# CMU-SAFARI/Scrooge

Hardware: AMD Instinct MI355X
Metric: aligned pairs/s (+ GCUPS) at W=64, 10kb reads; 1/2/4/8 MI355X (higher is better)
Workload: dtype u64

## Files before the change

### scrooge_amd/csrc/genasm_lane_kernel.hip

```cpp

#include <hip/hip_runtime.h>
#include <stdint.h>
#include <type_traits>

#include "lane_common.h"

namespace scrg {

constexpr int LANE_TB_COLS = 31;
constexpr uint32_t LANE_RING_BYTES = 68;
constexpr uint32_t LANE_SCRATCH_BYTES = 36;
constexpr uint32_t LANE_EQ_BYTES = 32;
constexpr uint32_t LANE_NOMATCH_BYTES = 8;
constexpr uint32_t LANE_WAVE_LDS_BYTES = 64u * (LANE_RING_BYTES + LANE_SCRATCH_BYTES + LANE_EQ_BYTES + LANE_NOMATCH_BYTES);
constexpr uint32_t LANE_EQ_SLOT_STRIDE = 512;
constexpr uint32_t LANE_EQ_REGION_BYTES = 4u * LANE_EQ_SLOT_STRIDE;
constexpr uint32_t LANE_EQ_FIELD_MASK = 3u * LANE_EQ_SLOT_STRIDE;
constexpr uint32_t LANE_REST_BYTES = LANE_WAVE_LDS_BYTES - LANE_EQ_REGION_BYTES;
constexpr int LANE_EQ_AHEAD = 8;

__device__ __forceinline__ uint32_t lane_read_offset(uint32_t fwd_offset, uint32_t read_idx, uint32_t read_len, uint32_t revm)
{
    return bitop3<TT_BFI>(sub_sat_u32(read_len - read_idx, 64u), fwd_offset, revm);
}
__device__ __forceinline__ void lane_pattern_rev(const Planes pw, uint32_t left, uint32_t revm, bool any_rev, uint64_t& rlo, uint64_t& rhi)
{
    rlo = brev64(pw.lo);
    rhi = brev64(pw.hi);
    if (any_rev) {
        const uint32_t sh = sub_sat_u32(64u, left);
        const uint64_t flo = ~(pw.lo << sh), fhi = ~(pw.hi << sh);
        rlo = ((uint64_t)bitop3<TT_BFI>((uint32_t)(flo >> 32), (uint32_t)(rlo >> 32), revm) << 32) | bitop3<TT_BFI>((uint32_t)flo, (uint32_t)rlo, revm);
        rhi = ((uint64_t)bitop3<TT_BFI>((uint32_t)(fhi >> 32), (uint32_t)(rhi >> 32), revm) << 32) | bitop3<TT_BFI>((uint32_t)fhi, (uint32_t)rhi, revm);
    }
}

constexpr uint32_t LANE_TEXT_REV = 1u << 7;
__device__ __forceinline__ uint32_t lane_text_offset(uint32_t ref_idx, uint32_t text_len, uint32_t tr_in)
{
    return bitop3<TT_BFI>(text_rev_at(text_len, ref_idx, 0u).at, ref_idx, neg_mask(tr_in << 24));
}
__device__ __forceinline__ void lane_text_rev(Planes& tw, uint32_t text_len, uint32_t ref_idx, uint32_t tr_in)
{
    const uint32_t tm = neg_mask(tr_in << 24);
    const uint32_t sh = text_rev_at(text_len, ref_idx, 0u).sh;
    const uint64_t flo = ~brev64(tw.lo << sh), fhi = ~brev64(tw.hi << sh);
    tw.lo = ((uint64_t)bitop3<TT_BFI>((uint32_t)(flo >> 32), (uint32_t)(tw.lo >> 32), tm) << 32) | bitop3<TT_BFI>((uint32_t)flo, (uint32_t)tw.lo, tm);
    tw.hi = ((uint64_t)bitop3<TT_BFI>((uint32_t)(fhi >> 32), (uint32_t)(tw.hi >> 32), tm) << 32) | bitop3<TT_BFI>((uint32_t)fhi, (uint32_t)tw.hi, tm);
}

template <bool NOMATCH>
__device__ __forceinline__ void lane_write_eq(const uint64_t rlo, const uint64_t rhi, const uint32_t iv0, const uint32_t iv1,
                                              const uint32_t eq_b, const uint32_t nomatch_b)
{
    const uint32_t rl0 = (uint32_t)rlo, rl1 = (uint32_t)(rlo >> 32), rh0 = (uint32_t)rhi, rh1 = (uint32_t)(rhi >> 32);
    lds_write64(eq_b, make_uint2(~(rl0 | rh0) | iv0, ~(rl1 | rh1) | iv1));
    lds_write64(eq_b + LANE_EQ_SLOT_STRIDE, make_uint2((rl0 & ~rh0) | iv0, (rl1 & ~rh1) | iv1));
    lds_write64(eq_b + 2u * LANE_EQ_SLOT_STRIDE, make_uint2((~rl0 & rh0) | iv0, (~rl1 & rh1) | iv1));
    lds_write64(eq_b + 3u * LANE_EQ_SLOT_STRIDE, make_uint2((rl0 & rh0) | iv0, (rl1 & rh1) | iv1));
    if (NOMATCH) lds_write64(nomatch_b, make_uint2(iv0, iv1));
}
struct LaneEqAddr {
    uint32_t xe0, xo0, xe1, xo1, eq_b;
    __device__ __forceinline__ LaneEqAddr(const Planes tw, const uint32_t eq_b_) : eq_b(eq_b_)
    {
        const uint32_t tl0 = (uint32_t)tw.lo, tl1 = (uint32_t)(tw.lo >> 32), th0 = (uint32_t)tw.hi, th1 = (uint32_t)(tw.hi >> 32);
        xe0 = bitop3<TT_BFI>(tl0, th0 << 1, 0x55555555u), xo0 = bitop3<TT_BFI>(th0, tl0 >> 1, 0xaaaaaaaau);
        xe1 = bitop3<TT_BFI>(tl1, th1 << 1, 0x55555555u), xo1 = bitop3<TT_BFI>(th1, tl1 >> 1, 0xaaaaaaaau);
    }
    __device__ __forceinline__ uint32_t at(const int i) const
    {
        const int b = i & 31;
        const uint32_t x = (b & 1) ? (i < 32 ? xo0 : xo1) : (i < 32 ? xe0 : xe1);
        const int f = (b & 1) ? b - 1 : b;
        const uint32_t u = f >= 9 ? x >> (f - 9) : x << (9 - f);
        return bitop3<TT_ANDOR>(u, LANE_EQ_FIELD_MASK, eq_b);
    }
};

template <bool SHORT_N>
__device__ __forceinline__ void lane_window_table(const Planes tw, const uint64_t rlo, const uint64_t rhi, const uint32_t n, const uint32_t m,
                                                  const uint32_t stop, uint64_t (&tab)[LANE_TB_COLS],
                                                  const uint32_t eq_b, const uint32_t nomatch_b, const bool write_eq = true)
{
    const uint64_t valid = ~0ull << (64u - m);
    const uint32_t iv0 = ~(uint32_t)valid, iv1 = ~(uint32_t)(valid >> 32);
    if (write_eq) lane_write_eq<SHORT_N>(rlo, rhi, iv0, iv1, eq_b, nomatch_b);
    const LaneEqAddr ea(tw, eq_b);
    auto eq_addr = [&](int i) -> uint32_t {
        const uint32_t a = ea.at(i);
        if (!SHORT_N) return a;
        return bitop3<TT_BFI>(a, nomatch_b, neg_mask((uint32_t)i - n));
    };
    uint2 eqw[LANE_EQ_AHEAD];
#pragma unroll
    for (int k = 0; k < LANE_EQ_AHEAD; k++) eqw[k] = lds_read64(eq_addr(63 - k));
    uint32_t pv0 = (uint32_t)valid, pv1 = (uint32_t)(valid >> 32), mv0 = 0u, mv1 = 0u;
#pragma unroll
    for (int i = 63; i >= 0; i--) {
        const uint2 eq_now = eqw[(63 - i) % LANE_EQ_AHEAD];
        if (i - LANE_EQ_AHEAD >= 0) eqw[(63 - i) % LANE_EQ_AHEAD] = lds_read64(eq_addr(i - LANE_EQ_AHEAD));
        {
            const uint32_t eq0 = eq_now.x, eq1 = eq_now.y;
            const uint32_t xv0 = eq0 | mv0, xv1 = eq1 | mv1;
            const uint32_t t0 = eq0 & pv0, t1 = eq1 & pv1;
            const uint64_t sum = add64(((uint64_t)t1 << 32) | t0, ((uint64_t)pv1 << 32) | pv0);
            const uint32_t xh0 = bitop3<TT_XH>((uint32_t)sum, pv0, eq0), xh1 = bitop3<TT_XH>((uint32_t)(sum >> 32), pv1, eq1);
            const uint32_t ph0 = bitop3<TT_PH>(mv0, xh0, pv0), ph1 = bitop3<TT_PH>(mv1, xh1, pv1);
            const uint32_t mh0 = pv0 & xh0, mh1 = pv1 & xh1;
            const uint64_t phs = shl1(((uint64_t)ph1 << 32) | ph0);
            const uint64_t mhs = shl1(((uint64_t)mh1 << 32) | mh0);
            pv0 = bitop3<TT_PVN>((uint32_t)mhs, xv0, (uint32_t)phs);
            pv1 = bitop3<TT_PVN>((uint32_t)(mhs >> 32), xv1, (uint32_t)(phs >> 32));
            mv0 = (uint32_t)phs & xv0;
            mv1 = (uint32_t)(phs >> 32) & xv1;
            if (i < LANE_TB_COLS)
                tab[i] = ((uint64_t)bitop3<TT_NOR3>(pv1, ph1, stop) << 32) | bitop3<TT_V0>(pv1, ph1, xh1);
        }
    }
}

constexpr int BAND_UP = 10, BAND_DOWN = 21, BAND_SAFE = 19;
static_assert(BAND_UP + BAND_DOWN + 1 == 32 && BAND_SAFE / 2 + 1 <= BAND_UP && BAND_SAFE + 1 <= BAND_DOWN, "the band holds every cell a safe walk asks about");
constexpr int TT_D0 = bitop3_table([](int sum, int pv, int xv) { return (sum ^ pv) | xv; });
constexpr int TT_OR3 = bitop3_table([](int a, int b, int c) { return a | b | c; });
constexpr int TT_NIV_BAND = bitop3_table([](int v1, int v0, int stop) { return ~(v1 & v0) | stop; });
__device__ __forceinline__ uint64_t lane_band_stop0(const uint32_t TBL)
{
    uint64_t s0 = 0x8000000000000000ull >> (TBL + (uint32_t)BAND_UP - 1u);
    asm volatile("" : "+s"(s0));
    return s0;
}
__device__ __forceinline__ uint32_t lane_band_stop(const uint64_t stop0, const int i)
{
    return (uint32_t)((stop0 << i) >> 32);
}
constexpr bool LANE_BAND_TABLE = true;
constexpr uint32_t BAND_STRETCH = 32, BAND_REDO_MAX = 6;
__device__ __forceinline__ uint32_t add_masked(uint32_t acc, const uint32_t x, const uint32_t mask)
{
    uint32_t t;
    asm volatile("v_and_b32 %0, %2, %3\n\tv_add_u32 %1, %1, %0" : "=&v"(t), "+v"(acc) : "s"(mask), "v"(x));
    return acc;
}
__device__ __forceinline__ uint32_t lane_window_table_band(const Planes tw, const uint64_t rlo, const uint64_t rhi, const uint32_t TBL,
                                                           uint64_t (&tab)[LANE_TB_COLS], const uint32_t eq_b)
{
    lane_write_eq<false>(rlo, rhi, 0u, 0u, eq_b, 0u);
    const LaneEqAddr ea(tw, eq_b);
    const uint64_t stop0 = lane_band_stop0(TBL);
    auto band_eq = [&](const uint2 w, const int i) -> uint32_t {
        const int s = 62 - i - BAND_DOWN;
        if (s >= 32) return w.y >> (s - 32);
        if (s > 0) return __builtin_amdgcn_alignbit(w.y, w.x, (uint32_t)s);
        if (s == 0) return w.x;
        return __builtin_amdgcn_alignbit(w.x, 0xffffffffu, (uint32_t)(32 + s));
    };
    uint2 eqw[LANE_EQ_AHEAD];
#pragma unroll
    for (int k = 0; k < LANE_EQ_AHEAD; k++) eqw[k] = lds_read64(ea.at(63 - k));
    uint32_t pv = ~0u << (BAND_DOWN + 1), mv = 0u;
    uint32_t fd = 0u;
#pragma unroll
    for (int i = 63; i >= 0; i--) {
        const uint32_t eq = band_eq(eqw[(63 - i) % LANE_EQ_AHEAD], i);
        if (i - LANE_EQ_AHEAD >= 0) eqw[(63 - i) % LANE_EQ_AHEAD] = lds_read64(ea.at(i - LANE_EQ_AHEAD));
        const uint32_t xv = eq | mv;
        const uint32_t d0 = bitop3<TT_D0>((eq & pv) + pv, pv, xv);
        const uint32_t ph = bitop3<TT_PH>(mv, d0, pv);
        const uint32_t mh = pv & d0;
        fd = add_masked(fd, d0, 1u << (32 - BAND_UP));
        const uint32_t xvs = xv >> 1;
        pv = bitop3<TT_PVN>(mh, xvs, ph);
        mv = ph & xvs;
        if (i < LANE_TB_COLS) {
            uint32_t pv2;
            asm("v_add_u32 %0, %1, %1" : "=v"(pv2) : "v"(pv));
            uint32_t v1 = bitop3<TT_OR3>(pv2, ph, lane_band_stop(stop0, i)), v0 = bitop3<TT_V0>(pv2, ph, d0);
            asm volatile("" : "+v"(v1), "+v"(v0));
            tab[i] = ((uint64_t)v1 << 32) | v0;
        }
    }
    return 64u - (fd >> (32 - BAND_UP));
}

template <int OUT>
__global__ __launch_bounds__(256, 4) void genasm_lane_kernel(AlignArgs a)
{
    constexpr bool EDITS = OUT == LANE_OUT_EDITS, NONE = OUT == LANE_OUT_NONE;
    constexpr bool BAND = LANE_BAND_TABLE;
    constexpr uint32_t REST_BYTES = NONE ? 64u * LANE_NOMATCH_BYTES : LANE_REST_BYTES;
    constexpr uint32_t STAGE_BYTES = NONE ? 0u : 64u * (LANE_RING_BYTES + LANE_SCRATCH_BYTES);
    extern __shared__ __attribute__((aligned(16))) uint32_t lds[];
    char* const lds_b = reinterpret_cast<char*>(lds);

    const uint32_t lane = threadIdx.x & 63u;
    const uint32_t wave = threadIdx.x >> 6, wpg = blockDim.x >> 6;
    const uint32_t wave_b = wpg * LANE_EQ_REGION_BYTES + wave * REST_BYTES;
    const uint32_t ring_b = wave_b + lane * LANE_RING_BYTES;
    const uint32_t scr_b = wave_b + 64u * LANE_RING_BYTES + lane * LANE_SCRATCH_BYTES;
    uint8_t* const lds8 = reinterpret_cast<uint8_t*>(lds);
    const uint32_t lds0 = (uint32_t)(uintptr_t)(__attribute__((address_space(3))) char*)lds_b;
    const uint32_t eq_b = lds0 + wave * LANE_EQ_REGION_BYTES + lane * 8u;
    const uint32_t nomatch_b = lds0 + wave_b + STAGE_BYTES + lane * LANE_NOMATCH_BYTES;
    const uint32_t W = (uint32_t)a.W;
    const uint32_t TBL = (uint32_t)a.tb_limit;

    bool has_pair = false;
    uint32_t pair = 0;
    const uint64_t* text_w = a.seq;
    const uint64_t* read_w = a.seq;
    uint32_t tr_in = 0;
    uint64_t cigar_off = 0;
    uint32_t text_len = 0, read_len = 0, cigar_cap = 0;
    uint32_t ref_idx = 0, read_idx = 0, edits = 0;
    uint32_t lim = 0xffffffffu;
    uint32_t revm = 0;
    int32_t nr = -1;
    uint32_t flushed = 0;
    uint32_t pos = 0;
    uint32_t mbase = 0;
    WindowWords twords = {0, 0, 0, 0}, pwords = {0, 0, 0, 0};
    bool queue_empty = false;
    const bool timing = SCRG_TIMING(a);
    uint64_t cy_fetch = 0, cy_setup = 0, cy_dc = 0, cy_tb = 0, cy_p1 = 0;
    uint32_t st_rounds = 0, st_gen = 0;
    uint32_t band_ctl = 0;
    uint32_t st_band = 0, st_redone = 0, st_skipped = 0;
    const uint64_t rt0 = timing ? __builtin_amdgcn_s_memrealtime() : 0;

    auto write_piece = [&]() {
        if constexpr (!NONE) scrg::write_piece<EDITS>(a, lds, ring_b, cigar_off, cigar_cap, flushed, !SCRG_ABL(a, 16));
    };
    auto flush_pieces = [&]() {
        if constexpr (!NONE) {
            const bool need = has_pair && (EDITS ? pos - flushed >= 32u : nr - (int32_t)flushed >= 15);
            if (__any(need)) {
                if (need) write_piece();
            }
        }
    };
    auto ring_guard = [&](uint32_t fill, uint32_t limit) {
        if (__any(has_pair && fill >= limit)) {
            if (has_pair && fill >= (EDITS ? 32u : 16u)) write_piece();
        }
    };

    uint32_t rot = hw_wave_slot();
    for (;;) {
        if (!SCRG_SW(a, 1)) rotate_priority(rot++);
        const uint64_t tm0 = timing ? __builtin_readcyclecounter() : 0;
        for (;;) {
            const bool over = has_pair && edits > lim;
            const bool fin = over || (has_pair && read_idx >= read_len);
            if (__any(fin)) {
                if (over) abandon_pair<OUT>(a, pair, edits);
                else if constexpr (NONE) { if (fin) retire_pair_distance(a, pair, edits, ref_idx); }
                else if (fin) retire_pair<EDITS>(a, lds, ring_b, pair, cigar_off, cigar_cap, flushed, EDITS ? pos : (uint32_t)(nr + 1), nr, edits, !SCRG_ABL(a, 16));
                has_pair = has_pair && !fin;
            }
            const bool want = !has_pair && !queue_empty;
            if (!__any(want)) break;
            const uint32_t idx = claim_pairs(a, lane, want);
            const bool got = want && idx < a.n_pairs;
            if (__any(want && idx >= a.n_pairs)) queue_empty = true;
            if (got) {
                const scrg_pair_desc pd = a.pairs[idx];
                pair = idx;
                const TextStretch ts = text_stretch(pd.text_off, pd.text_len, a.text_rev != 0u, a.text_stride);
                text_w = a.seq + (ts.off >> 5);
                const uint64_t r_off = a.stranded ? pd.read_off & ~SCRG_READ_REVCOMP : pd.read_off;
                revm = (a.stranded && (pd.read_off & SCRG_READ_REVCOMP)) ? 0xffffffffu : 0u;
                read_w = a.seq + (r_off >> 5);
                tr_in = ((uint32_t)ts.off & 31u) | (((uint32_t)r_off & 31u) << 8) | (ts.rev ? LANE_TEXT_REV : 0u);
                text_len = ts.len;
                read_len = (uint32_t)pd.read_len;
                lim = pair_edit_limit(a, read_len);
                if constexpr (NONE) {
                    ref_idx = read_idx = edits = 0;
                } else {
                    cigar_off = pd.cigar_off;
                    cigar_cap = pd.cigar_cap > 0xffffffffull ? 0xffffffffu : (uint32_t)pd.cigar_cap;
                    ref_idx = read_idx = edits = flushed = pos = mbase = 0;
                    nr = -1;
                }
                has_pair = true;
                twords = load_window_words_at(text_w, tr_in & 31u, ts.rev ? text_rev_at(text_len, 0u, 0u).at : 0u, a.text_stride);
                pwords = load_window_words_at(read_w, tr_in >> 8, lane_read_offset(0u, 0u, read_len, revm), a.read_stride);
            }
        }
        if (!__any(has_pair)) break;
        const bool wave_rev = a.stranded && __any(has_pair && revm != 0u);
        const bool wave_trev = a.text_rev && __any(has_pair && (tr_in & LANE_TEXT_REV) != 0u);

        const uint64_t tm1 = timing ? __builtin_readcyclecounter() : 0;
        const uint32_t n = has_pair ? min(W, sub_sat_u32(text_len, ref_idx)) : 0u;
        const uint32_t m = has_pair ? min(W, read_len - read_idx) : 1u;
        Planes tw = window_planes(twords);
        const Planes pw = window_planes(pwords);
        if (wave_trev) lane_text_rev(tw, text_len, ref_idx, tr_in);
        asm volatile("" :: "v"(tw.lo), "v"(tw.hi), "v"(pw.lo), "v"(pw.hi) : "memory");
        flush_pieces();
        const uint64_t tm2 = timing ? __builtin_readcyclecounter() : 0;

        uint64_t tab[LANE_TB_COLS];
        const uint32_t jlim = has_pair ? min(m, TBL) : 0u;
        const uint32_t stop = 0x80000000u >> jlim;
        const bool short_n = __any(has_pair && n != 64u);
        uint64_t rlo, rhi;
        lane_pattern_rev(pw, read_len - read_idx, revm, wave_rev, rlo, rhi);
        uint32_t j = 0, ti, nDm = 0, Xm = 0, nIm = 0;
        auto walk = [&](auto full_tag, auto band_tag) {
            constexpr bool FULL = decltype(full_tag)::value;
            constexpr bool BANDED = decltype(band_tag)::value;
            const uint64_t stop0 = BANDED ? lane_band_stop0(TBL) : 0ull;
#pragma unroll
            for (int i = 0; i < LANE_TB_COLS; i++) {
                if (!FULL && (uint32_t)i >= TBL) continue;
                const uint32_t x = (BANDED ? bitop3<TT_NIV_BAND>((uint32_t)(tab[i] >> 32), (uint32_t)tab[i], lane_band_stop(stop0, i))
                                           : bitop3<TT_NIV>((uint32_t)(tab[i] >> 32), (uint32_t)tab[i], stop)) << j;
                const uint32_t ni = ffbh_u32(x);
                if constexpr (!NONE) lds_store_u8(lds0 + scr_b + (uint32_t)i, ni);
                nIm = __builtin_amdgcn_alignbit(nIm, x, 31);
                j += ni;
                const uint64_t both = tab[i] << j;
                const uint32_t nt1 = (uint32_t)(both >> 32), t0 = (uint32_t)both;
                nDm = __builtin_amdgcn_alignbit(nDm, nt1, 31);
                Xm = __builtin_amdgcn_alignbit(Xm, t0, 31);
                if (BANDED) j += neg_mask(nt1);
                else j -= neg_mask(nt1);
            }
        };
        bool walked = false, eq_written = false;
        uint64_t tm3 = 0;
        if constexpr (BAND) {
            if (W == 64u && !short_n && !__any(has_pair && m != 64u) && !SCRG_SEL(a.debug, SCRG_SWITCH_NO_BAND) && !SCRG_ABL(a, 2) && !SCRG_ABL(a, 8)) {
                if ((band_ctl >> 16) != 0u) {
                    band_ctl -= 1u << 16;
                    st_skipped++;
                } else {
                    const uint32_t d_band = lane_window_table_band(tw, rlo, rhi, TBL, tab, eq_b);
                    walked = !__any(has_pair && d_band > (uint32_t)BAND_SAFE);
                    eq_written = true;
                    st_band++;
                    st_redone += walked ? 0u : 1u;
                    band_ctl += walked ? 1u : 0x101u;
                    if (((band_ctl >> 8) & 15u) > BAND_REDO_MAX && !SCRG_SEL(a.debug, SCRG_SWITCH_BAND_ALWAYS)) {
                        const uint32_t fails = (band_ctl >> 12) & 15u;
                        band_ctl = (32u << (16u + fails)) | (min(fails + 1u, 6u) << 12);
                    } else if ((band_ctl & 255u) == BAND_STRETCH) {
                        band_ctl = 0u;
                    }
                    if (walked) {
                        tm3 = timing ? __builtin_readcyclecounter() : 0;
                        j = (uint32_t)BAND_UP - 1u;
                        if (TBL == (uint32_t)LANE_TB_COLS) walk(std::true_type{}, std::true_type{});
                        else walk(std::false_type{}, std::true_type{});
                        j = has_pair ? j + TBL - ((uint32_t)BAND_UP - 1u) : 0u;
                        nDm = has_pair ? ~nDm : 0u;
                        nIm = has_pair ? nIm : ~0u;
                    }
                }
            }
        }
        if (!walked) {
            if (SCRG_ABL(a, 2)) {
#pragma unroll
                for (int i = 0; i < LANE_TB_COLS; i++) tab[i] = ((uint64_t)~stop << 32) | (((uint32_t)tw.lo * (uint32_t)(i + 1)) | stop);
            } else if (short_n) {
                lane_window_table<true>(tw, rlo, rhi, n, m, stop, tab, eq_b, nomatch_b);
                st_gen++;
            } else {
                lane_window_table<false>(tw, rlo, rhi, n, m, stop, tab, eq_b, nomatch_b, !eq_written);
            }
            tm3 = timing ? __builtin_readcyclecounter() : 0;
            if (SCRG_ABL(a, 8)) { j = jlim; nDm = ~0u; }
            else if (TBL == (uint32_t)LANE_TB_COLS) walk(std::true_type{}, std::false_type{});
            else walk(std::false_type{}, std::false_type{});
        }
        {
            if (timing) cy_p1 += __builtin_readcyclecounter() - tm3;
            const uint32_t TBc = min(TBL, (uint32_t)LANE_TB_COLS);
            const uint32_t nsh = 32u - TBc;
            const uint32_t notD = nDm << nsh, Xraw = Xm << nsh;
            const uint32_t Draw = ~notD;
            const uint32_t Im = ~nIm << nsh;
            const uint32_t ti_stopped = (31u - ffbl_u32((notD >> 1) | Im)) & 31u;
            ti = bitop3<TT_BFI>(TBc, ti_stopped, neg_mask(j - jlim));
            const uint32_t A = ~(0xffffffffu >> ti);
            const uint32_t D = Draw & A, X = Xraw & A;
            const uint32_t B = ((D ^ (D >> 1)) | (X ^ (X >> 1)) | Im | 0x80000000u) & A;
            const uint32_t nD = (uint32_t)__builtin_popcount(D), nX = (uint32_t)__builtin_popcount(X);
            edits += j - ti + 2u * nD + nX;
            ref_idx += ti;
            read_idx += j;
            twords = load_window_words_at(text_w, tr_in & 31u, wave_trev ? lane_text_offset(ref_idx, text_len, tr_in) : ref_idx, a.text_stride);
            const uint32_t left_x = read_idx ^ read_len;
            const uint32_t fwd_at = read_idx & neg_mask(left_x | (0u - left_x));
            pwords = load_window_words_at(read_w, tr_in >> 8, wave_rev ? lane_read_offset(fwd_at, read_idx, read_len, revm) : fwd_at, a.read_stride);

            if constexpr (NONE) {
                (void)B;
            } else if constexpr (EDITS) {
                uint32_t E = SCRG_ABL(a, 4) ? 0u : (D | X | Im);
                nr += (int32_t)(__builtin_popcount(B) + __builtin_popcount(Im));
                uint32_t c = ffbh_u32(E);
                uint32_t ni = lds8[scr_b + c];
                auto put = [&](uint32_t at, uint32_t b) { lds8[ring_b + (at & 63u)] = (uint8_t)b; };
                auto event = [&]() {
                    const uint32_t sh = 31u - c;
                    const uint32_t bit = 0x80000000u >> (c & 31u);
                    uint32_t iB = __builtin_amdgcn_ubfe(Im, sh, 1), dx = __builtin_amdgcn_ubfe(D | X, sh, 1);
                    const uint32_t xB = __builtin_amdgcn_ubfe(X, sh, 1);
                    const uint32_t t = mbase + c;
                    E = bitop3<TT_ANDN>(E, bit, bit);
                    const uint32_t nx = ffbh_u32(E);
                    const uint32_t step = 0xC0u - 0x80u * xB;
                    const bool side = ni * iB > 3u;
                    if (__any(side)) {
                        if (side) {
                            auto emit = [&](uint32_t b) {
                                put(pos, b);
                                pos++;
                                if (pos - flushed >= 32u) write_piece();
                            };
                            emit(0x80u | t);
                            for (uint32_t q = 1; q < ni; q++) emit(0x80u);
                            mbase = 0u - c;
                            if (dx) {
                                emit(step);
                                mbase = ~c;
                            }
                            iB = dx = 0;
                        }
                    }
                    put(pos, 0x80u | t);
                    put(pos + 1u, 0x80u);
                    put(pos + 2u, 0x80u);
                    pos += iB ? ni : 0u;
                    put(pos, step | (iB ? 0u : t));
                    pos += dx;
                    mbase = dx ? ~c : (iB ? 0u - c : mbase);
                    ni = lds8[scr_b + nx];
                    c = nx;
                };
                uint32_t trips = 0;
                while (__any(E != 0u)) {
                    if (trips >= 2u) ring_guard(pos - flushed, 50u);
                    event();
                    event();
                    trips++;
                }
                put(pos, mbase + ti);
                pos += has_pair ? 1u : 0u;
                mbase = 0;
            } else {
            uint32_t E = SCRG_ABL(a, 4) ? 0u : (B | Im);
            uint32_t c0 = ffbh_u32(E);
            E = bitop3<TT_ANDN>(E, 0x80000000u >> (c0 & 31u), 0u);
            uint32_t c1 = ffbh_u32(E);
            uint32_t q = 2u * (uint32_t)nr + 2u;
            auto event = [&](uint32_t& c, const uint32_t ni, const uint32_t nx) {
                const uint32_t sh = 31u - c;
                const uint32_t aI = ring_b + (q & 62u);
                q = add_twice(q, __builtin_amdgcn_ubfe(Im, sh, 1));
                const uint32_t w = add3(mad24(__builtin_amdgcn_ubfe(X, sh, 1), 27u << 8, mad24(__builtin_amdgcn_ubfe(D, sh, 1), 7u << 8, sh)),
                                        min(nx, ti), ((uint32_t)'=' << 8) - 31u);
                const uint32_t aS = ring_b + (q & 62u);
                q = add_twice(q, __builtin_amdgcn_ubfe(B, sh, 1));
                E = bitop3<TT_ANDN>(E, 0x80000000u >> (nx & 31u), 0u);
                c = ffbh_u32(E);
                *reinterpret_cast<uint16_t*>(lds_b + aI) = (uint16_t)(((uint32_t)'I' << 8) | ni);
                *reinterpret_cast<uint16_t*>(lds_b + aS) = (uint16_t)w;
            };
            auto trip = [&]() {
                const uint32_t n0 = lds8[scr_b + c0], n1 = lds8[scr_b + c1];
                event(c0, n0, c1);
                event(c1, n1, c0);
            };
            for (uint32_t trips = 0; trips < 4u && __any(c0 < 32u); trips++) trip();
            while (__any(c0 < 32u)) {
                ring_guard((q >> 1) - flushed, 27u);
                trip();
            }
            nr = ((int32_t)q >> 1) - 1;
            }
        }
        st_rounds++;
        if (timing) {
            const uint64_t tm4 = __builtin_readcyclecounter();
            cy_fetch += tm1 - tm0;
            cy_setup += tm2 - tm1;
            cy_dc += tm3 - tm2;
            cy_tb += tm4 - tm3;
        }
    }
    if (timing && lane == 0) {
        atomicAdd((unsigned long long*)&a.stats[0], (unsigned long long)st_rounds | ((unsigned long long)st_skipped << 32));
        atomicAdd((unsigned long long*)&a.stats[1], (unsigned long long)st_gen | ((unsigned long long)st_band << 21) | ((unsigned long long)st_redone << 42));
        atomicAdd((unsigned long long*)&a.stats[2], (unsigned long long)cy_p1);
        atomicAdd((unsigned long long*)&a.stats[3], (unsigned long long)cy_fetch);
        atomicAdd((unsigned long long*)&a.stats[4], (unsigned long long)cy_setup);
        atomicAdd((unsigned long long*)&a.stats[5], (unsigned long long)cy_dc);
        atomicAdd((unsigned long long*)&a.stats[6], (unsigned long long)cy_tb);
        const uint64_t rt1 = __builtin_amdgcn_s_memrealtime();
        atomicAdd((unsigned long long*)&a.stats[7], (unsigned long long)(rt1 - rt0));
        atomicMax((unsigned long long*)&a.stats[8], (unsigned long long)rt0);
        atomicMax((unsigned long long*)&a.stats[9], (unsigned long long)((1ull << 62) - rt0));
        atomicMax((unsigned long long*)&a.stats[10], (unsigned long long)rt1);
        atomicMax((unsigned long long*)&a.stats[11], (unsigned long long)((1ull << 62) - rt1));
    }
}

constexpr uint32_t SPLIT_FIELDS = 6;
constexpr uint32_t SPLIT_BUF_BYTES = SPLIT_FIELDS * 256u + 64u * LANE_SCRATCH_BYTES;
constexpr uint32_t SPLIT_PAIR_LDS_BYTES = 64u * (LANE_RING_BYTES + LANE_EQ_BYTES + LANE_NOMATCH_BYTES) + 2u * SPLIT_BUF_BYTES;
constexpr uint32_t SPLIT_WG_LDS_BYTES = 4u * SPLIT_PAIR_LDS_BYTES + 64u;
constexpr uint32_t SPLIT_VALID = 1u << 8, SPLIT_FIRST = 1u << 9, SPLIT_LAST = 1u << 10;
constexpr uint32_t SPLIT_OVER = 1u << 11;

__global__ __launch_bounds__(512, 2) void genasm_lane_split_kernel(AlignArgs a)
{
    extern __shared__ __attribute__((aligned(16))) uint32_t lds[];
    char* const lds_b = reinterpret_cast<char*>(lds);
    uint8_t* const lds8 = reinterpret_cast<uint8_t*>(lds);
    const uint32_t lane = threadIdx.x & 63u;
    const uint32_t wave = threadIdx.x >> 6, duo = wave & 3u;
    const bool consumer = wave >= 4u;
    const uint32_t duo_b = 4u * LANE_EQ_REGION_BYTES + duo * (SPLIT_PAIR_LDS_BYTES - LANE_EQ_REGION_BYTES);
    const uint32_t ring_b = duo_b + lane * LANE_RING_BYTES;
    const uint32_t lds0 = (uint32_t)(uintptr_t)(__attribute__((address_space(3))) char*)lds_b;
    const uint32_t eq_b = lds0 + duo * LANE_EQ_REGION_BYTES + lane * 8u;
    const uint32_t nomatch_b = lds0 + duo_b + 64u * LANE_RING_BYTES + lane * LANE_NOMATCH_BYTES;
    const uint32_t bufs_b = duo_b + 64u * (LANE_RING_BYTES + LANE_NOMATCH_BYTES);
    const uint32_t flags_w = (4u * SPLIT_PAIR_LDS_BYTES) >> 2;
    const uint32_t W = (uint32_t)a.W;
    const uint32_t TBL = (uint32_t)a.tb_limit;
    const uint32_t TBc = min(TBL, (uint32_t)LANE_TB_COLS);
    const uint32_t nsh = 32u - TBc;
    auto rec_w = [&](uint32_t buf, uint32_t field) -> uint32_t { return ((bufs_b + buf * SPLIT_BUF_BYTES) >> 2) + field * 64u + lane; };
    auto len_b = [&](uint32_t buf) -> uint32_t { return bufs_b + buf * SPLIT_BUF_BYTES + SPLIT_FIELDS * 256u + lane * LANE_SCRATCH_BYTES; };
    auto all_done = [&](uint32_t r) -> bool {
        const uint32_t f = flags_w + (r & 1u) * 4u;
        return (lds[f] & lds[f + 1] & lds[f + 2] & lds[f + 3]) != 0u;
    };

    if (!consumer) {
        bool has_pair = false, active = true;
        uint32_t pair = 0;
        uint64_t text_off = 0, read_off = 0;
        uint32_t text_len = 0, read_len = 0;
        uint32_t ref_idx = 0, read_idx = 0, edits = 0;
        uint32_t lim = 0xffffffffu;
        uint32_t revm = 0;
        bool trev = false;
        WindowWords twords = {0, 0, 0, 0}, pwords = {0, 0, 0, 0};
        bool queue_empty = false;
        uint32_t st_rounds = 0;
        const uint32_t slot = hw_wave_slot();
        for (uint32_t r = 0;; r++) {
            const uint32_t buf = r & 1u;
            uint32_t first = 0;
            if (active) {
                if (!SCRG_SW(a, 1)) rotate_priority(r + slot);
                has_pair = has_pair && read_idx < read_len && edits <= lim;
                for (;;) {
                    const bool want = !has_pair && !queue_empty;
                    if (!__any(want)) break;
                    const uint32_t idx = claim_pairs(a, lane, want);
                    const bool got = want && idx < a.n_pairs;
                    if (__any(want && idx >= a.n_pairs)) queue_empty = true;
                    if (got) {
                        const LanePair p = unpack_pair(a, idx);
                        pair = idx;
                        text_off = p.text_off;
                        read_off = p.read_off;
                        revm = p.rev ? 0xffffffffu : 0u;
                        trev = p.trev;
                        text_len = p.text_len;
                        read_len = p.read_len;
                        lim = pair_edit_limit(a, p.read_len);
                        ref_idx = read_idx = edits = 0;
                        has_pair = true;
                        first = SPLIT_FIRST;
                        twords = load_window_words(a.seq, text_off, trev ? text_rev_at(text_len, 0u, 0u).at : 0u, a.text_stride);
                        pwords = load_window_words(a.seq, read_off, lane_read_offset(0u, 0u, read_len, revm), a.read_stride);
                    }
                }
                if (!__any(has_pair)) active = false;
            }
            if (active) {
                const bool live = has_pair && read_idx < read_len;
                const uint32_t n = (live && ref_idx < text_len) ? min(W, text_len - ref_idx) : 0u;
                const uint32_t m = live ? min(W, read_len - read_idx) : 1u;
                Planes tw = {0, 0}, pw = {0, 0};
                if (live) {
                    tw = window_planes(twords);
                    pw = window_planes(pwords);
                }
                const bool wave_trev = a.text_rev && __any(live && trev);
                if (wave_trev) lane_text_rev(tw, text_len, ref_idx, trev ? LANE_TEXT_REV : 0u);
                uint64_t tab[LANE_TB_COLS];
                const uint32_t jlim = live ? min(m, TBL) : 0u;
                const uint32_t stop = 0x80000000u >> jlim;
                const bool short_n = __any(live && n != 64u);
                const bool wave_rev = a.stranded && __any(live && revm != 0u);
                uint64_t rlo, rhi;
                lane_pattern_rev(pw, read_len - read_idx, revm, wave_rev, rlo, rhi);
                if (short_n) lane_window_table<true>(tw, rlo, rhi, n, m, stop, tab, eq_b, nomatch_b);
                else lane_window_table<false>(tw, rlo, rhi, n, m, stop, tab, eq_b, nomatch_b);
                uint32_t j = 0, nDm = 0, Xm = 0, nIm = 0;
                const uint32_t lb = len_b(buf);
                auto walk = [&](auto full_tag) {
                    constexpr bool FULL = decltype(full_tag)::value;
#pragma unroll
                    for (int i = 0; i < LANE_TB_COLS; i++) {
                        if (!FULL && (uint32_t)i >= TBL) continue;
                        const uint32_t x = bitop3<TT_NIV>((uint32_t)(tab[i] >> 32), (uint32_t)tab[i], stop) << j;
                        const uint32_t ni = ffbh_u32(x);
                        lds_store_u8(lds0 + lb + (uint32_t)i, ni);
                        nIm = __builtin_amdgcn_alignbit(nIm, x, 31);
                        j += ni;
                        const uint64_t both = tab[i] << j;
                        const uint32_t nt1 = (uint32_t)(both >> 32), t0 = (uint32_t)both;
                        nDm = __builtin_amdgcn_alignbit(nDm, nt1, 31);
                        Xm = __builtin_amdgcn_alignbit(Xm, t0, 31);
                        j -= neg_mask(nt1);
                    }
                };
                if (TBL == (uint32_t)LANE_TB_COLS) walk(std::true_type{});
                else walk(std::false_type{});
                const uint32_t notD = nDm << nsh, Xraw = Xm << nsh;
                const uint32_t Im = ~nIm << nsh;
                const uint32_t ti_stopped = (31u - ffbl_u32((notD >> 1) | Im)) & 31u;
                const uint32_t ti = bitop3<TT_BFI>(TBc, ti_stopped, neg_mask(j - jlim));
                const uint32_t A = ~(0xffffffffu >> ti);
                const uint32_t D = ~notD & A, X = Xraw & A;
                edits += j - ti + 2u * (uint32_t)__builtin_popcount(D) + (uint32_t)__builtin_popcount(X);
                ref_idx += ti;
                read_idx += j;
                twords = load_window_words(a.seq, text_off, wave_trev ? lane_text_offset(ref_idx, text_len, trev ? LANE_TEXT_REV : 0u) : ref_idx, a.text_stride);
                const uint32_t left_x = read_idx ^ read_len;
                pwords = load_window_words(a.seq, read_off, lane_read_offset(read_idx & neg_mask(left_x | (0u - left_x)), read_idx, read_len, revm), a.read_stride);
                const uint32_t over = (has_pair && edits > lim) ? SPLIT_OVER : 0u;
                const uint32_t last = (has_pair && (read_idx >= read_len || over)) ? SPLIT_LAST : 0u;
                lds[rec_w(buf, 0)] = D;
                lds[rec_w(buf, 1)] = X;
                lds[rec_w(buf, 2)] = Im;
                lds[rec_w(buf, 3)] = ti | (has_pair ? SPLIT_VALID : 0u) | first | last | over;
                lds[rec_w(buf, 4)] = pair;
                lds[rec_w(buf, 5)] = edits;
                st_rounds++;
            } else {
                lds[rec_w(buf, 3)] = 0u;
            }
            if (lane == 0) lds[flags_w + buf * 4u + duo] = active ? 0u : 1u;
            __syncthreads();
            if (all_done(r)) break;
        }
        if (SCRG_TIMING(a) && lane == 0) atomicAdd((unsigned long long*)&a.stats[0], (unsigned long long)st_rounds);
        return;
    }

    bool open = false;
    uint32_t pair = 0;
    uint64_t cigar_off = 0;
    uint32_t cigar_cap = 0;
    int32_t nr = -1;
    uint32_t flushed = 0;
    auto flush_pieces = [&]() {
        const bool need = open && nr - (int32_t)flushed >= 16;
        if (__any(need)) {
            if (need) write_piece<false>(a, lds, ring_b, cigar_off, cigar_cap, flushed);
        }
    };
    auto consume = [&](uint32_t buf) {
        const uint32_t meta = lds[rec_w(buf, 3)];
        if (!__any((meta & SPLIT_VALID) != 0u)) return;
        const bool valid = (meta & SPLIT_VALID) != 0u;
        const uint32_t ti = meta & 31u;
        const uint32_t D = valid ? lds[rec_w(buf, 0)] : 0u, X = valid ? lds[rec_w(buf, 1)] : 0u, Im = valid ? lds[rec_w(buf, 2)] : 0u;
        if (valid && (meta & SPLIT_FIRST)) {
            pair = lds[rec_w(buf, 4)];
            const LanePair p = unpack_pair(a, pair);
            cigar_off = p.cigar_off;
            cigar_cap = p.cigar_cap;
            nr = -1;
            flushed = 0;
            open = true;
        }
        const uint32_t A = ~(0xffffffffu >> ti);
        const uint32_t B = ((D ^ (D >> 1)) | (X ^ (X >> 1)) | Im | 0x80000000u) & A;
        const uint32_t scr_b = len_b(buf);
        uint32_t E = valid ? (B | Im) : 0u;
        uint32_t c = ffbh_u32(E);
        uint32_t ni = lds8[scr_b + c];
        uint32_t q = 2u * (uint32_t)nr + 2u;
        auto event = [&]() {
            const uint32_t sh = 31u - c;
            const uint32_t bit = 0x80000000u >> (c & 31u);
            *reinterpret_cast<uint16_t*>(lds_b + ring_b + (q & 62u)) = (uint16_t)(((uint32_t)'I' << 8) | ni);
            q = add_twice(q, __builtin_amdgcn_ubfe(Im, sh, 1));
            E = bitop3<TT_ANDN>(E, bit, bit);
            const uint32_t nx = ffbh_u32(E);
            ni = lds8[scr_b + nx];
            const uint32_t w = add3(mad24(__builtin_amdgcn_ubfe(X, sh, 1), 27u << 8, mad24(__builtin_amdgcn_ubfe(D, sh, 1), 7u << 8, sh)),
                                    min(nx, ti), ((uint32_t)'=' << 8) - 31u);
            *reinterpret_cast<uint16_t*>(lds_b + ring_b + (q & 62u)) = (uint16_t)w;
            q = add_twice(q, __builtin_amdgcn_ubfe(B, sh, 1));
            c = nx;
        };
        uint32_t trips = 0;
        while (__any(E != 0u)) {
            event();
            event();
            if (++trips == 3u) {
                trips = 0;
                nr = ((int32_t)q >> 1) - 1;
                flush_pieces();
            }
        }
        nr = ((int32_t)q >> 1) - 1;
        flush_pieces();
        const bool fin = valid && (meta & SPLIT_LAST) != 0u;
        if (__any(fin)) {
            if (fin && (meta & SPLIT_OVER)) {
                abandon_pair<LANE_OUT_RUNS>(a, pair, lds[rec_w(buf, 5)]);
                open = false;
            } else if (fin) {
                const uint32_t n_runs = (uint32_t)(nr + 1);
                while (n_runs - flushed >= 16u) write_piece<false>(a, lds, ring_b, cigar_off, cigar_cap, flushed);
                const uint32_t rem = n_runs - flushed;
                const uint32_t rd = (ring_b >> 2) + ((flushed & 16u) >> 1);
                uint32_t* const dst = reinterpret_cast<uint32_t*>(a.runs + cigar_off + flushed);
                for (uint32_t k = 0; 2u * k < rem; k++)
                    if (flushed + 2u * k < cigar_cap) dst[k] = lds[rd + k];
                a.ed[pair] = (int64_t)lds[rec_w(buf, 5)];
                a.n_runs[pair] = n_runs;
                a.status[pair] = n_runs > cigar_cap ? LANE_STATUS_OVERFLOW : LANE_STATUS_DONE;
                open = false;
            }
        }
    };
    for (uint32_t r = 0;; r++) {
        if (r != 0u) consume((r - 1u) & 1u);
        __syncthreads();
        if (all_done(r)) {
            consume(r & 1u);
            break;
        }
    }
}

hipError_t launch_align_lane_split(const AlignArgs& a, int grid, hipStream_t s)
{
    const dim3 g((grid + 3) / 4), b(512);
    hipLaunchKernelGGL(genasm_lane_split_kernel, g, b, SPLIT_WG_LDS_BYTES, s, a);
    return hipGetLastError();
}

hipError_t launch_align_lane(const AlignArgs& a, int grid, size_t lds_bytes, hipStream_t s, LaneOutput out)
{
    const unsigned wpg = SCRG_SW(a, 64) ? 1u : (SCRG_SW(a, 128) ? 2u : 4u);
    const dim3 g((grid + wpg - 1) / wpg), b(64 * wpg);
    with_lane_output(out, [&](auto o) { hipLaunchKernelGGL(genasm_lane_kernel<decltype(o)::value>, g, b, wpg * lds_bytes, s, a); });
    return hipGetLastError();
}

}
```

### scrooge_amd/csrc/genasm_lane_mw_kernel.hip

```cpp

#include <hip/hip_runtime.h>
#include <stdint.h>

#include "lane_multiword.h"
#include "row_ops.h"

namespace scrg {

namespace {

constexpr uint32_t MW_RING_BYTES = 68;

}

template <int NW, int RW, int OUT>
__global__ __launch_bounds__(64) void genasm_lane_mw_kernel(AlignArgs a)
{
    extern __shared__ __attribute__((aligned(16))) uint32_t lds[];
    char* const lds_b = reinterpret_cast<char*>(lds);
    uint8_t* const lds8 = reinterpret_cast<uint8_t*>(lds);

    constexpr bool EDITS = OUT == LANE_OUT_EDITS, NONE = OUT == LANE_OUT_NONE;
    const uint32_t lane = threadIdx.x;
    const uint32_t W = (uint32_t)a.W;
    const uint32_t TBL = (uint32_t)a.tb_limit;
    const uint32_t ring_b = lane * MW_RING_BYTES;
    const uint32_t len_b = 64u * MW_RING_BYTES + lane * lane_mw_len_bytes(a.tb_limit);
    uint64_t* const tab = reinterpret_cast<uint64_t*>(a.spill) + (uint64_t)blockIdx.x * (uint64_t)TBL * 2u * RW * 64u + lane;

    bool rev = false;
    bool trev = false;
    LaneWork lp;

    auto write_piece = [&]() {
        if constexpr (!NONE) scrg::write_piece<EDITS>(a, lds, ring_b, lp.cigar_off, lp.cigar_cap, lp.flushed);
    };
    auto flush_pieces = [&]() {
        for (;;) {
            const bool need = lp.has_pair && lp.nr + 1 - (int32_t)lp.flushed >= 16;
            if (!__any(need)) break;
            if (need) write_piece();
        }
    };
    auto push_run = [&](uint32_t op, uint32_t count) {
        lp.nr++;
        *reinterpret_cast<uint16_t*>(lds_b + ring_b + (((uint32_t)lp.nr & 31u) << 1)) = (uint16_t)(count | (op << 8));
    };
    auto emit = [&](uint32_t b) {
        lds8[ring_b + (lp.pos & 63u)] = (uint8_t)b;
        lp.pos++;
        if (lp.pos - lp.flushed >= 32u) write_piece();
    };

    for (;;) {
        if (!next_pairs<OUT, !EDITS>(a, lds, ring_b, lane, lp, rev, trev)) break;

        const uint32_t n = (lp.has_pair && lp.ref_idx < lp.text_len) ? min(W, lp.text_len - lp.ref_idx) : 0u;
        const uint32_t m = lp.has_pair ? min(W, lp.read_len - lp.read_idx) : 1u;
        uint64_t tlo[NW], thi[NW], rlo[NW], rhi[NW], valid[NW];
        const bool wave_trev = a.text_rev && __any(lp.has_pair && trev);
#pragma unroll
        for (int w = 0; w < NW; w++) {
            Planes t = {0, 0}, p = {0, 0};
            if (lp.has_pair && !trev && 64u * (uint32_t)w < n) t = load_window_strided(a.seq, lp.text_off, lp.ref_idx + 64u * (uint32_t)w, a.text_stride);
            if (wave_trev) {
                if (lp.has_pair && trev && 64u * (uint32_t)w < n) t = text_revcomp_word(a.seq, lp.text_off, lp.text_len, lp.ref_idx, (uint32_t)w, a.text_stride);
            }
            if (lp.has_pair && 64u * (uint32_t)w < m) p = load_window_strided(a.seq, lp.read_off, lp.read_idx + 64u * (uint32_t)w, a.read_stride);
            tlo[w] = t.lo;
            thi[w] = t.hi;
            rlo[w] = brev64(p.lo);
            rhi[w] = brev64(p.hi);
            if (a.stranded && __any(lp.has_pair && rev)) {
                const Planes rv = revcomp_pattern_word(a.seq, lp.read_off, lp.read_len, lp.has_pair ? lp.read_idx : lp.read_len, (uint32_t)w, a.read_stride);
                if (lp.has_pair && rev) { rlo[w] = rv.lo; rhi[w] = rv.hi; }
            }
            const uint32_t lo = 64u * (uint32_t)w;
            valid[w] = m >= lo + 64u ? ~0ull : (m <= lo ? 0ull : ~0ull << (64u - (m - lo)));
        }
        const uint32_t jlim = lp.has_pair ? min(m, TBL) : 0u;
        const Row<RW> stop = row_bit<RW>(jlim);

        {
            uint64_t pv[NW], mv[NW];
#pragma unroll
            for (int w = 0; w < NW; w++) { pv[w] = valid[w]; mv[w] = 0; }
#pragma unroll
            for (int wi = NW - 1; wi >= 0; wi--) {
                for (int b = 63; b >= 0; b--) {
                    const uint32_t i = 64u * (uint32_t)wi + (uint32_t)b;
                    if (i >= W) continue;
                    const uint64_t sl = 0ull - ((tlo[wi] >> b) & 1ull), sh = 0ull - ((thi[wi] >> b) & 1ull);
                    const bool in_text = i < n;
                    uint64_t xv[NW], xh[NW], ph[NW], mh[NW];
                    uint64_t carry = 0;
#pragma unroll
                    for (int w = NW - 1; w >= 0; w--) {
                        const uint64_t eq = (in_text ? ~((rlo[w] ^ sl) | (rhi[w] ^ sh)) : 0ull) | ~valid[w];
                        xv[w] = eq | mv[w];
                        const uint64_t t = eq & pv[w];
                        const uint64_t s1 = t + pv[w];
                        const uint64_t s2 = s1 + carry;
                        carry = (uint64_t)(s1 < t) | (uint64_t)(s2 < s1);
                        xh[w] = (s2 ^ pv[w]) | eq;
                        ph[w] = mv[w] | ~(xh[w] | pv[w]);
                        mh[w] = pv[w] & xh[w];
                    }
#pragma unroll
                    for (int w = 0; w < NW; w++) {
                        const uint64_t ph1 = (ph[w] << 1) | (w + 1 < NW ? ph[w + 1] >> 63 : 0ull);
                        const uint64_t mh1 = (mh[w] << 1) | (w + 1 < NW ? mh[w + 1] >> 63 : 0ull);
                        pv[w] = mh1 | ~(xv[w] | ph1);
                        mv[w] = ph1 & xv[w];
                    }
                    if (i < TBL) {
#pragma unroll
                        for (int r = 0; r < RW; r++) {
                            const uint64_t pvr = r < NW ? pv[r < NW ? r : 0] : 0ull, phr = r < NW ? ph[r < NW ? r : 0] : 0ull, xhr = r < NW ? xh[r < NW ? r : 0] : ~0ull;
                            tab[((uint64_t)(i * 2u) * RW + r) * 64u] = ~((pvr | phr) | stop.w[r]);
                            tab[((uint64_t)(i * 2u + 1u) * RW + r) * 64u] = (pvr | ~(phr | xhr)) | stop.w[r];
                        }
                    }
                }
            }
        }

        {
            uint32_t j = 0;
            Row<RW> nDm = row_zero<RW>(), Xm = row_zero<RW>(), nIm = row_zero<RW>();
            constexpr int CH = RW == 1 ? 16 : (RW == 2 ? 8 : 4);
            for (uint32_t i0 = 0; i0 < TBL; i0 += CH) {
                Row<RW> nv1[CH], v0[CH];
#pragma unroll
                for (int q = 0; q < CH; q++) {
                    const uint32_t i = min(i0 + (uint32_t)q, TBL - 1u);
#pragma unroll
                    for (int r = 0; r < RW; r++) {
                        nv1[q].w[r] = tab[((uint64_t)(i * 2u) * RW + r) * 64u];
                        v0[q].w[r] = tab[((uint64_t)(i * 2u + 1u) * RW + r) * 64u];
                    }
                }
#pragma unroll
                for (int q = 0; q < CH; q++) {
                    const uint32_t i = i0 + (uint32_t)q;
                    if (i >= TBL) continue;
                    Row<RW> x;
#pragma unroll
                    for (int r = 0; r < RW; r++) x.w[r] = nv1[q].w[r] | ~v0[q].w[r] | stop.w[r];
                    x = row_shl<RW>(x, j);
                    const uint32_t ni = row_clz<RW>(x);
                    if constexpr (!NONE) lds8[len_b + i] = (uint8_t)ni;
                    nIm = row_shl1_in<RW>(nIm, x.w[0] >> 63);
                    j += ni;
                    const Row<RW> nt1 = row_shl<RW>(nv1[q], j), t0 = row_shl<RW>(v0[q], j);
                    nDm = row_shl1_in<RW>(nDm, nt1.w[0] >> 63);
                    Xm = row_shl1_in<RW>(Xm, t0.w[0] >> 63);
                    j += (uint32_t)(nt1.w[0] >> 63);
                }
            }
            const uint32_t nsh = 64u * RW - TBL;
            Row<RW> Draw = row_shl<RW>(nDm, nsh), Im;
            const Row<RW> Xraw = row_shl<RW>(Xm, nsh);
#pragma unroll
            for (int r = 0; r < RW; r++) { Draw.w[r] = ~Draw.w[r]; Im.w[r] = ~nIm.w[r]; }
            Im = row_shl<RW>(Im, nsh);
            const Row<RW> lim = row_bit<RW>(TBL);
            Row<RW> dead;
#pragma unroll
            for (int r = 0; r < RW; r++) dead.w[r] = (Draw.w[r] & Xraw.w[r]) | lim.w[r];
            const uint32_t ti = row_clz<RW>(dead);
            const Row<RW> A = row_top<RW>(ti);
            Row<RW> D, X, B, E;
#pragma unroll
            for (int r = 0; r < RW; r++) { D.w[r] = Draw.w[r] & A.w[r]; X.w[r] = Xraw.w[r] & A.w[r]; }
            const Row<RW> D1 = row_shr1<RW>(D), X1 = row_shr1<RW>(X);
#pragma unroll
            for (int r = 0; r < RW; r++) {
                B.w[r] = ((D.w[r] ^ D1.w[r]) | (X.w[r] ^ X1.w[r]) | Im.w[r] | (r == 0 ? TOP : 0ull)) & A.w[r];
                E.w[r] = B.w[r] | Im.w[r];
            }
            lp.edits += j - ti + 2u * row_pop<RW>(D) + row_pop<RW>(X);
            lp.ref_idx += ti;
            lp.read_idx += j;

            if constexpr (NONE) {
            } else if constexpr (EDITS) {
                Row<RW> Ev;
#pragma unroll
                for (int r = 0; r < RW; r++) Ev.w[r] = D.w[r] | X.w[r] | Im.w[r];
                lp.nr += (int32_t)(row_pop<RW>(B) + row_pop<RW>(Im));
                while (__any(row_any<RW>(Ev))) {
                    if (row_any<RW>(Ev)) {
                        const uint32_t c = row_clz<RW>(Ev);
                        const Row<RW> bit = row_bit<RW>(c);
#pragma unroll
                        for (int r = 0; r < RW; r++) Ev.w[r] &= ~bit.w[r];
                        uint32_t t = lp.mbase + c;
                        if (row_test<RW>(Im, c)) {
                            const uint32_t ni = lds8[len_b + c];
                            for (; t >= 63u; t -= 63u) emit(0x3Fu);
                            emit(0x80u | t);
                            for (uint32_t q = 1; q < ni; q++) emit(0x80u);
                            t = 0;
                            lp.mbase = 0u - c;
                        }
                        const bool isD = row_test<RW>(D, c), isX = row_test<RW>(X, c);
                        if (isD || isX) {
                            for (; t >= 63u; t -= 63u) emit(0x3Fu);
                            emit((isX ? 0x40u : 0xC0u) | t);
                            lp.mbase = ~c;
                        }
                    }
                }
                if (__any(lp.has_pair)) {
                    if (lp.has_pair) {
                        uint32_t t = lp.mbase + ti;
                        for (; t >= 63u; t -= 63u) emit(0x3Fu);
                        emit(t);
                    }
                }
                lp.mbase = 0;
            } else
            while (__any(row_any<RW>(E))) {
                if (row_any<RW>(E)) {
                    const uint32_t c = row_clz<RW>(E);
                    if (row_test<RW>(Im, c)) push_run((uint32_t)'I', lds8[len_b + c]);
                    const Row<RW> bit = row_bit<RW>(c);
#pragma unroll
                    for (int r = 0; r < RW; r++) E.w[r] &= ~bit.w[r];
                    const uint32_t nx = min(row_clz<RW>(E), ti);
                    if (row_test<RW>(B, c))
                        push_run(row_test<RW>(D, c) ? (uint32_t)'D' : (row_test<RW>(X, c) ? (uint32_t)'X' : (uint32_t)'='), nx - c);
                }
                flush_pieces();
            }
        }
    }
}

template <int NW, int RW> static hipError_t launch_mw(const AlignArgs& a, int grid, size_t lds_bytes, hipStream_t s, LaneOutput out)
{
    with_lane_output(out, [&](auto o) { hipLaunchKernelGGL((genasm_lane_mw_kernel<NW, RW, decltype(o)::value>), dim3(grid), dim3(64), lds_bytes, s, a); });
    return hipGetLastError();
}

hipError_t launch_align_lane_mw(const AlignArgs& a, int grid, size_t lds_bytes, hipStream_t s, LaneOutput out)
{
    const int nw = a.W <= 64 ? 1 : (a.W <= 128 ? 2 : 4), rw = a.tb_limit / 64 + 1;
    if (nw == 1 && rw == 1) return launch_mw<1, 1>(a, grid, lds_bytes, s, out);
    if (nw == 1 && rw == 2) return launch_mw<1, 2>(a, grid, lds_bytes, s, out);
    if (nw == 2 && rw == 3) return launch_mw<2, 3>(a, grid, lds_bytes, s, out);
    if (nw == 2 && rw == 1) return launch_mw<2, 1>(a, grid, lds_bytes, s, out);
    if (nw == 2 && rw == 2) return launch_mw<2, 2>(a, grid, lds_bytes, s, out);
    if (nw == 4 && rw == 1) return launch_mw<4, 1>(a, grid, lds_bytes, s, out);
    if (nw == 4 && rw == 2) return launch_mw<4, 2>(a, grid, lds_bytes, s, out);
    if (nw == 4 && rw == 3) return launch_mw<4, 3>(a, grid, lds_bytes, s, out);
    if (nw == 4 && rw == 4) return launch_mw<4, 4>(a, grid, lds_bytes, s, out);
    return hipErrorInvalidValue;
}

}
```

### scrooge_amd/csrc/genasm_lane_parts_kernel.hip

```cpp

#include <hip/hip_runtime.h>
#include <stdint.h>
#include <type_traits>

#include "lane_multiword.h"

namespace scrg {

namespace {

constexpr int PT_COLS = 16;
constexpr uint32_t PT_RING_BYTES = 68;
constexpr uint32_t PT_SCRATCH_BYTES = 20;
constexpr int PT_EQ_AHEAD = 2;

__device__ __forceinline__ uint64_t pt_from_row(uint64_t w0, uint64_t w1, uint32_t s)
{
    const bool far = s >= 64u;
    const uint64_t hi = far ? w1 : w0, lo = far ? 0ull : w1;
    const uint32_t b = s & 63u;
    return shl64(hi, b) | shr64(lo >> 1, 63u - b);
}

template <int NW, bool STORE, bool SHORT>
__device__ __forceinline__ void pt_sweep16(LaneVec<NW>& st, const uint32_t xe, const uint32_t xo, const int32_t nrel, const uint2 (&stop)[2],
                                           uint64_t (&tab)[PT_COLS][2][2], const uint32_t eq_b, const uint32_t nomatch_b)
{
    constexpr int SLOT_SHIFT = NW == 2 ? 4 : 5;
    auto eq_addr = [&](int c) -> uint32_t {
        const uint32_t x = (c & 1) ? xo : xe;
        const int f = (c & 1) ? c - 1 : c;
        const uint32_t u = f >= SLOT_SHIFT ? x >> (f - SLOT_SHIFT) : x << (SLOT_SHIFT - f);
        const uint32_t a = bitop3<TT_ANDOR>(u, 3u << SLOT_SHIFT, eq_b);
        return (!SHORT || c < nrel) ? a : nomatch_b;
    };
    uint2 eqw[PT_EQ_AHEAD][NW];
#pragma unroll
    for (int k = 0; k < PT_EQ_AHEAD; k++) {
        const uint32_t ad = eq_addr(PT_COLS - 1 - k);
#pragma unroll
        for (int q = 0; q < NW; q++) eqw[k][q] = lds_read64(ad + 8u * q);
    }
#pragma unroll
    for (int c = PT_COLS - 1; c >= 0; c--) {
        uint2 eq[NW];
#pragma unroll
        for (int q = 0; q < NW; q++) eq[q] = eqw[(PT_COLS - 1 - c) % PT_EQ_AHEAD][q];
        if (c - PT_EQ_AHEAD >= 0) {
            const uint32_t ad = eq_addr(c - PT_EQ_AHEAD);
#pragma unroll
            for (int q = 0; q < NW; q++) eqw[(PT_COLS - 1 - c) % PT_EQ_AHEAD][q] = lds_read64(ad + 8u * q);
        }
        const LaneColumn<NW> col = sweep_column<NW>(st, eq);
        if (STORE) {
#pragma unroll
            for (int r = 0; r < 2; r++) {
                table_words<NW>(st, col, r, stop[r], tab[c][0][r], tab[c][1][r]);
            }
        }
    }
}

}

template <int NW, int OUT>
__global__ __launch_bounds__(256, 2) void genasm_lane_parts_kernel(AlignArgs a)
{
    extern __shared__ __attribute__((aligned(16))) uint32_t lds[];
    char* const lds_b = reinterpret_cast<char*>(lds);
    uint8_t* const lds8 = reinterpret_cast<uint8_t*>(lds);
    constexpr uint32_t SLOT = NW == 2 ? 16u : 32u;
    constexpr uint32_t EQ_BYTES = 4u * SLOT, NOMATCH_BYTES = SLOT, TEXT_BYTES = 16u * NW;
    constexpr bool EDITS = OUT == LANE_OUT_EDITS, NONE = OUT == LANE_OUT_NONE;
    constexpr uint32_t STAGE_BYTES = NONE ? 0u : PT_RING_BYTES + PT_SCRATCH_BYTES;
    constexpr uint32_t WAVE_LDS = 64u * (STAGE_BYTES + EQ_BYTES + NOMATCH_BYTES + TEXT_BYTES);
    constexpr uint32_t CP_DWORDS = 4u * NW;

    const uint32_t lane = threadIdx.x & 63u;
    const uint32_t wave_b = (threadIdx.x >> 6) * WAVE_LDS;
    const uint32_t ring_b = wave_b + lane * PT_RING_BYTES;
    const uint32_t scr_b = wave_b + 64u * PT_RING_BYTES + lane * PT_SCRATCH_BYTES;
    const uint32_t eq_base = (uint32_t)(uintptr_t)(__attribute__((address_space(3))) char*)lds_b + wave_b + 64u * STAGE_BYTES;
    const uint32_t eq_b = eq_base + lane * EQ_BYTES;
    const uint32_t nomatch_b = eq_base + 64u * EQ_BYTES + lane * NOMATCH_BYTES;
    const uint32_t text_b = eq_base + 64u * (EQ_BYTES + NOMATCH_BYTES) + lane * TEXT_BYTES;
    const uint32_t swz = NW == 2 ? (lane >> 2) & 3u : (lane >> 1) & 3u;
    const uint32_t W = (uint32_t)a.W;
    const uint32_t TBL = (uint32_t)a.tb_limit;
    const uint32_t P = (TBL + (uint32_t)PT_COLS - 1u) / (uint32_t)PT_COLS;
    const int32_t ktop = (int32_t)((W + (uint32_t)PT_COLS - 1u) / (uint32_t)PT_COLS) - 1;
    uint32_t* const cps = a.spill + ((uint64_t)blockIdx.x * 4u + (threadIdx.x >> 6)) * 8u * CP_DWORDS * 64u + lane;

    bool rev = false;
    bool trev = false;
    LaneWork lp;
    const LaneLds ll = {lds, ring_b, scr_b};
    uint32_t st_rounds = 0;

    auto flush_pieces = [&]() {
        if constexpr (!NONE) for (;;) {
            const bool need = lp.has_pair && (EDITS ? lp.pos - lp.flushed >= 32u : lp.nr - (int32_t)lp.flushed >= 16);
            if (!__any(need)) break;
            if (need) write_piece<EDITS>(a, lds, ring_b, lp.cigar_off, lp.cigar_cap, lp.flushed);
        }
    };

    auto save_checkpoint = [&](uint32_t k, const LaneVec<NW>& st) {
        uint32_t* const dst = cps + (uint64_t)k * CP_DWORDS * 64u;
#pragma unroll
        for (int q = 0; q < NW; q++) {
            dst[(4 * q + 0) * 64] = st.pv[q].x;
            dst[(4 * q + 1) * 64] = st.pv[q].y;
            dst[(4 * q + 2) * 64] = st.mv[q].x;
            dst[(4 * q + 3) * 64] = st.mv[q].y;
        }
    };
    auto load_checkpoint = [&](uint32_t k, LaneVec<NW>& st) {
        const uint32_t* const src = cps + (uint64_t)k * CP_DWORDS * 64u;
#pragma unroll
        for (int q = 0; q < NW; q++) {
            st.pv[q] = make_uint2(src[(4 * q + 0) * 64], src[(4 * q + 1) * 64]);
            st.mv[q] = make_uint2(src[(4 * q + 2) * 64], src[(4 * q + 3) * 64]);
        }
    };

    uint32_t rot = hw_wave_slot();
    for (;;) {
        if (!SCRG_SW(a, 1)) rotate_priority(rot++);
        if (!next_pairs<OUT>(a, lds, ring_b, lane, lp, rev, trev)) break;
        const bool has_pair = lp.has_pair;

        const LaneWindow ext = window_extent(lp, W, TBL);
        const uint32_t n = ext.n, jlim = ext.jlim;
        uint2 stop[2];
        {
            const uint64_t sb = 0x8000000000000000ull >> (jlim & 63u);
            const uint64_t s0 = jlim < 64u ? sb : 0ull, s1 = jlim < 64u ? 0ull : sb;
            stop[0] = make_uint2((uint32_t)s0, (uint32_t)(s0 >> 32));
            stop[1] = make_uint2((uint32_t)s1, (uint32_t)(s1 >> 32));
        }
        LaneVec<NW> st;
        {
            uint32_t tl[2 * NW], th[2 * NW];
            window_setup<NW, SLOT>(a, lp, rev, trev, ext, eq_b, nomatch_b, swz, st, tl, th);
#pragma unroll
            for (int q = 0; q < 2 * NW; q++) {
                const uint32_t l = tl[q], h = th[q];
                lds_write64(text_b + 8u * q, make_uint2(bitop3<TT_BFI>(l, h << 1, 0x55555555u), bitop3<TT_BFI>(h, l >> 1, 0xaaaaaaaau)));
            }
        }

        uint64_t tab[PT_COLS][2][2];
        auto sweep_chunk = [&](int32_t k, auto store_tag) {
            constexpr bool STORE = decltype(store_tag)::value;
            const int32_t nrel = (int32_t)n - (int32_t)PT_COLS * k;
            if (!__any(has_pair && nrel > 0)) {
                if (STORE) {
                    LaneVec<NW> keep = st;
                    pt_sweep16<NW, true, true>(keep, 0u, 0u, nrel, stop, tab, eq_b, nomatch_b);
                }
                return;
            }
            const uint2 xx = lds_read64(text_b + 8u * (uint32_t)(k >> 1));
            const uint32_t sh = (uint32_t)(k & 1) * 16u;
            const uint32_t xe = xx.x >> sh, xo = xx.y >> sh;
            if (__any(has_pair && nrel < PT_COLS)) pt_sweep16<NW, STORE, true>(st, xe, xo, nrel, stop, tab, eq_b, nomatch_b);
            else pt_sweep16<NW, STORE, false>(st, xe, xo, nrel, stop, tab, eq_b, nomatch_b);
        };
#pragma unroll 1
        for (int32_t k = ktop; k >= 1; k--) {
            if ((uint32_t)k < P) save_checkpoint((uint32_t)k, st);
            sweep_chunk(k, std::false_type{});
        }
        sweep_chunk(0, std::true_type{});
        constexpr bool PREFETCH = NW <= 3;
        if (PREFETCH && P > 1u) load_checkpoint(1u, st);

        uint32_t j = 0;
        uint32_t last_dx = 0;
        bool alive = has_pair;
#pragma unroll 1
        for (uint32_t part = 0; part < P; part++) {
            const uint32_t ncols = min((uint32_t)PT_COLS, TBL - (uint32_t)PT_COLS * part);
            if (part != 0u) {
                if (!__any(alive)) break;
                if (!PREFETCH) load_checkpoint(part, st);
                sweep_chunk((int32_t)part, std::true_type{});
                if (PREFETCH && part + 1u < P) load_checkpoint(part + 1u, st);
            }
            const uint32_t j0 = j;
            uint32_t nDm = 0, Xm = 0, nIm = 0;
            const uint64_t stop0 = ((uint64_t)stop[0].y << 32) | stop[0].x, stop1 = ((uint64_t)stop[1].y << 32) | stop[1].x;
            auto walk_part = [&](auto mode_tag) {
                constexpr int MODE = decltype(mode_tag)::value;
                nDm = Xm = nIm = 0;
                j = j0;
                if constexpr (MODE == 0) {
#pragma unroll
                    for (int s = 0; s < PT_COLS; s++) {
                        if ((uint32_t)s >= ncols) continue;
                        const uint64_t x0 = tab[s][0][0] | ~tab[s][1][0] | stop0, x1 = tab[s][0][1] | ~tab[s][1][1] | stop1;
                        const uint64_t top = pt_from_row(x0, x1, j);
                        const uint64_t nxt = j < 64u ? shl64(x1, j) : 0ull;
                        const uint32_t ni = (top != 0ull) ? clz64(top) : 64u + clz64(nxt);
                        if constexpr (!NONE) lds8[scr_b + s] = (uint8_t)ni;
                        nIm = __builtin_amdgcn_alignbit(nIm, (uint32_t)(top >> 32), 31);
                        j += ni;
                        const uint32_t nt1 = (uint32_t)(pt_from_row(tab[s][0][0], tab[s][0][1], j) >> 32);
                        const uint32_t t0 = (uint32_t)(pt_from_row(tab[s][1][0], tab[s][1][1], j) >> 32);
                        nDm = __builtin_amdgcn_alignbit(nDm, nt1, 31);
                        Xm = __builtin_amdgcn_alignbit(Xm, t0, 31);
                        j -= neg_mask(nt1);
                    }
                } else {
                    constexpr int WD = MODE - 1;
                    const uint64_t stopw = WD == 0 ? stop0 : stop1;
                    uint32_t jr = j - 64u * (uint32_t)WD;
#pragma unroll
                    for (int s = 0; s < PT_COLS; s++) {
                        if ((uint32_t)s >= ncols) continue;
                        const uint64_t x = tab[s][0][WD] | ~tab[s][1][WD] | stopw;
                        const uint64_t top = shl64(x, jr);
                        const uint32_t ni = min(ffbh_u32((uint32_t)(top >> 32)), min(ffbh_u32((uint32_t)top), 32u) + 32u);
                        if constexpr (!NONE) lds8[scr_b + s] = (uint8_t)ni;
                        nIm = __builtin_amdgcn_alignbit(nIm, (uint32_t)(top >> 32), 31);
                        jr += ni;
                        const uint32_t nt1 = (uint32_t)(shl64(tab[s][0][WD], jr) >> 32);
                        const uint32_t t0 = (uint32_t)(shl64(tab[s][1][WD], jr) >> 32);
                        nDm = __builtin_amdgcn_alignbit(nDm, nt1, 31);
                        Xm = __builtin_amdgcn_alignbit(Xm, t0, 31);
                        jr -= neg_mask(nt1);
                    }
                    j = jr + 64u * (uint32_t)WD;
                }
            };
            if (TBL <= 63u) {
                walk_part(std::integral_constant<int, 1>{});
            } else if (!__any(has_pair && j0 < 64u)) {
                walk_part(std::integral_constant<int, 2>{});
            } else if (!__any(has_pair && j0 > 40u)) {
                walk_part(std::integral_constant<int, 1>{});
                if (__any(has_pair && j > 63u)) walk_part(std::integral_constant<int, 0>{});
            } else {
                walk_part(std::integral_constant<int, 0>{});
            }
            const PartEvents ev = part_events<PT_COLS>(lp, has_pair, part == 0u, ncols, nDm, Xm, nIm, j - j0, last_dx, alive);
            if constexpr (EDITS) part_edits<PT_COLS, true, 2>(a, ll, ev, lp, flush_pieces);
            else if constexpr (!NONE) part_runs<PT_COLS, 3>(ll, ev, lp, flush_pieces);
            else (void)ev;
        }
        lp.read_idx += j;
        if constexpr (EDITS) {
            window_end_bytes<true>(ll, lp);
            flush_pieces();
        }
        st_rounds++;
    }
    if (SCRG_TIMING(a) && lane == 0) atomicAdd((unsigned long long*)&a.stats[0], (unsigned long long)st_rounds);
}

template <int NW> static void launch_parts(const AlignArgs& a, dim3 g, dim3 b, size_t lds, hipStream_t s, LaneOutput out)
{
    with_lane_output(out, [&](auto o) { hipLaunchKernelGGL((genasm_lane_parts_kernel<NW, decltype(o)::value>), g, b, lds, s, a); });
}

hipError_t launch_align_lane_parts(const AlignArgs& a, int grid, size_t lds_bytes, hipStream_t s, LaneOutput out)
{
    const dim3 g((grid + 3) / 4), b(256);
    const int nw = (a.W + 63) / 64;
    if (nw == 2) launch_parts<2>(a, g, b, 4 * lds_bytes, s, out);
    else if (nw == 3) launch_parts<3>(a, g, b, 4 * lds_bytes, s, out);
    else if (nw == 4) launch_parts<4>(a, g, b, 4 * lds_bytes, s, out);
    else return hipErrorInvalidValue;
    return hipGetLastError();
}

}
```

### scrooge_amd/csrc/genasm_lane_wide_kernel.hip

```cpp

#include <hip/hip_runtime.h>
#include <stdint.h>

#include "lane_multiword.h"

namespace scrg {

namespace {

#ifndef WD_BLOCKS_PER_CU
#define WD_BLOCKS_PER_CU 2
#endif
constexpr int WD_HALF = 32;
constexpr uint32_t WD_RING_BYTES = 68;
constexpr uint32_t WD_SCRATCH_BYTES = 36;
constexpr int WD_EQ_AHEAD = 8;

template <int NW> struct WdWindow {
    uint32_t tl[2 * NW], th[2 * NW];
    uint32_t n;
    uint2 stop;
};

template <int NW, int SHORT_N, int HI, int LO, int STORE>
__device__ __forceinline__ void wd_sweep(LaneVec<NW>& st, const WdWindow<NW>& w, uint64_t (&tab)[WD_HALF][2],
                                         const uint32_t eq_b, const uint32_t nomatch_b)
{
    uint32_t wtl[2 * NW], wth[2 * NW];
#pragma unroll
    for (int q = 0; q < 2 * NW; q++) {
        wtl[q] = w.tl[q];
        wth[q] = w.th[q];
        asm volatile("" : "+v"(wtl[q]), "+v"(wth[q]));
    }
    uint32_t xe[2 * NW], xo[2 * NW];
#pragma unroll
    for (int q = 0; q < 2 * NW; q++) {
        if (32 * q > HI || 32 * q + 31 < LO) continue;
        xe[q] = bitop3<TT_BFI>(wtl[q], wth[q] << 1, 0x55555555u);
        xo[q] = bitop3<TT_BFI>(wth[q], wtl[q] >> 1, 0xaaaaaaaau);
    }
    auto eq_addr = [&](int i) -> uint32_t {
        constexpr int SH = NW == 1 ? 3 : 4;
        const int b = i & 31;
        const uint32_t x = (b & 1) ? xo[i >> 5] : xe[i >> 5];
        const int f = (b & 1) ? b - 1 : b;
        const uint32_t u = f >= SH ? x >> (f - SH) : x << (SH - f);
        const uint32_t a = bitop3<TT_ANDOR>(u, 3u << SH, eq_b);
        if (SHORT_N == 0) return a;
        if (SHORT_N == 2) return bitop3<TT_BFI>(a, nomatch_b, neg_mask((uint32_t)i - w.n));
        return (uint32_t)i < w.n ? a : nomatch_b;
    };
    uint2 eqw[WD_EQ_AHEAD][NW];
#pragma unroll
    for (int k = 0; k < WD_EQ_AHEAD; k++) {
        if (HI - k < LO) continue;
        const uint32_t ad = eq_addr(HI - k);
#pragma unroll
        for (int q = 0; q < NW; q++) eqw[k][q] = lds_read64(ad + 8u * q);
    }
#pragma unroll
    for (int i = HI; i >= LO; i--) {
        uint2 eq[NW];
#pragma unroll
        for (int q = 0; q < NW; q++) eq[q] = eqw[(HI - i) % WD_EQ_AHEAD][q];
        if (i - WD_EQ_AHEAD >= LO) {
            const uint32_t ad = eq_addr(i - WD_EQ_AHEAD);
#pragma unroll
            for (int q = 0; q < NW; q++) eqw[(HI - i) % WD_EQ_AHEAD][q] = lds_read64(ad + 8u * q);
        }
        const LaneColumn<NW> col = sweep_column<NW>(st, eq);
        if (STORE >= 0 && i >= STORE && i < STORE + WD_HALF) {
            table_words<NW>(st, col, 0, w.stop, tab[i - STORE][0], tab[i - STORE][1]);
        }
    }
}

}

template <int NW, int OUT>
__global__ __launch_bounds__(256, WD_BLOCKS_PER_CU) void genasm_lane_wide_kernel(AlignArgs a)
{
    extern __shared__ __attribute__((aligned(16))) uint32_t lds[];
    char* const lds_b = reinterpret_cast<char*>(lds);
    uint8_t* const lds8 = reinterpret_cast<uint8_t*>(lds);
    constexpr bool EDITS = OUT == LANE_OUT_EDITS, NONE = OUT == LANE_OUT_NONE;
    constexpr uint32_t EQ_BYTES = 32u * NW, NOMATCH_BYTES = 8u * NW;
    constexpr uint32_t STAGE_BYTES = NONE ? 0u : WD_RING_BYTES + WD_SCRATCH_BYTES;
    constexpr uint32_t WAVE_LDS = 64u * (STAGE_BYTES + EQ_BYTES + NOMATCH_BYTES);

    const uint32_t lane = threadIdx.x & 63u;
    const uint32_t wave_b = (threadIdx.x >> 6) * WAVE_LDS;
    const uint32_t ring_b = wave_b + lane * WD_RING_BYTES;
    const uint32_t scr_b = wave_b + 64u * WD_RING_BYTES + lane * WD_SCRATCH_BYTES;
    const uint32_t eq_base = (uint32_t)(uintptr_t)(__attribute__((address_space(3))) char*)lds_b + wave_b + 64u * STAGE_BYTES;
    const uint32_t eq_b = eq_base + lane * EQ_BYTES;
    const uint32_t nomatch_b = eq_base + 64u * EQ_BYTES + lane * NOMATCH_BYTES;
    const uint32_t swz = NW == 1 ? (lane >> 3) & 3u : (lane >> 2) & 3u;
    const uint32_t W = (uint32_t)a.W;
    const uint32_t TBL = (uint32_t)a.tb_limit;
    const uint32_t HB = TBL - (uint32_t)WD_HALF;

    bool rev = false;
    bool trev = false;
    LaneWork lp;
    const LaneLds ll = {lds, ring_b, scr_b};
    uint32_t st_rounds = 0;

    auto flush_pieces = [&]() {
        if constexpr (!NONE) for (;;) {
            const bool need = lp.has_pair && (EDITS ? lp.pos - lp.flushed >= 32u : lp.nr - (int32_t)lp.flushed >= 16);
            if (!__any(need)) break;
            if (need) write_piece<EDITS>(a, lds, ring_b, lp.cigar_off, lp.cigar_cap, lp.flushed);
        }
    };

    uint32_t rot = hw_wave_slot();
    for (;;) {
        if (!SCRG_SW(a, 1)) rotate_priority(rot++);
        if (!next_pairs<OUT>(a, lds, ring_b, lane, lp, rev, trev)) break;
        const bool has_pair = lp.has_pair;

        const LaneWindow ext = window_extent(lp, W, TBL);
        const uint32_t n = ext.n;
        const uint64_t stop64 = 0x8000000000000000ull >> ext.jlim;
        WdWindow<NW> win;
        win.n = n;
        win.stop = make_uint2((uint32_t)stop64, (uint32_t)(stop64 >> 32));
        LaneVec<NW> st0;
        window_setup<NW, 8u * NW>(a, lp, rev, trev, ext, eq_b, nomatch_b, swz, st0, win.tl, win.th);
        const bool short_n = __any(has_pair && n < 64u);
        const bool short_pro = NW == 2 && __any(has_pair && n != ((W + 15u) & ~15u));
        uint64_t tab[WD_HALF][2];
        if constexpr (NW == 2) {
            if (W <= 80u) {
                if (short_pro) wd_sweep<NW, ((EDITS || NW == 2) ? 1 : 2), 79, 64, -1>(st0, win, tab, eq_b, nomatch_b);
                else wd_sweep<NW, 0, 79, 64, -1>(st0, win, tab, eq_b, nomatch_b);
            } else if (W <= 96u) {
                if (short_pro) wd_sweep<NW, ((EDITS || NW == 2) ? 1 : 2), 95, 64, -1>(st0, win, tab, eq_b, nomatch_b);
                else wd_sweep<NW, 0, 95, 64, -1>(st0, win, tab, eq_b, nomatch_b);
            } else if (W <= 112u) {
                if (short_pro) wd_sweep<NW, ((EDITS || NW == 2) ? 1 : 2), 111, 64, -1>(st0, win, tab, eq_b, nomatch_b);
                else wd_sweep<NW, 0, 111, 64, -1>(st0, win, tab, eq_b, nomatch_b);
            } else {
                if (short_pro) wd_sweep<NW, ((EDITS || NW == 2) ? 1 : 2), 127, 64, -1>(st0, win, tab, eq_b, nomatch_b);
                else wd_sweep<NW, 0, 127, 64, -1>(st0, win, tab, eq_b, nomatch_b);
            }
        }

        uint32_t j = 0;
        uint32_t last_dx = 0;
        bool alive = has_pair;
#pragma unroll 1
        for (int half = 0; half < 2; half++) {
            const uint32_t ncols = half == 0 ? (uint32_t)WD_HALF : HB;
            if (half == 1 && (HB == 0u || !__any(alive))) break;
            {
                LaneVec<NW> st = st0;
                if (half == 0) {
                    if (short_n) wd_sweep<NW, ((EDITS || NW == 2) ? 1 : 2), 63, 0, 0>(st, win, tab, eq_b, nomatch_b);
                    else wd_sweep<NW, 0, 63, 0, 0>(st, win, tab, eq_b, nomatch_b);
                } else {
                    if (short_n) wd_sweep<NW, ((EDITS || NW == 2) ? 1 : 2), 63, WD_HALF, WD_HALF>(st, win, tab, eq_b, nomatch_b);
                    else wd_sweep<NW, 0, 63, WD_HALF, WD_HALF>(st, win, tab, eq_b, nomatch_b);
                }
            }
            const uint32_t j0 = j;
            uint32_t nDm = 0, Xm = 0, nIm = 0;
#pragma unroll
            for (int s = 0; s < WD_HALF; s++) {
                if ((uint32_t)s >= ncols) continue;
                const uint32_t xl = bitop3<TT_NIV>((uint32_t)tab[s][0], (uint32_t)tab[s][1], win.stop.x);
                const uint32_t xu = bitop3<TT_NIV>((uint32_t)(tab[s][0] >> 32), (uint32_t)(tab[s][1] >> 32), win.stop.y);
                const uint64_t x = shl64(((uint64_t)xu << 32) | xl, j);
                const uint32_t ni = min(ffbh_u32((uint32_t)(x >> 32)), ffbh_u32((uint32_t)x) + 32u);
                if constexpr (!NONE) lds8[scr_b + s] = (uint8_t)ni;
                nIm = __builtin_amdgcn_alignbit(nIm, (uint32_t)(x >> 32), 31);
                j += ni;
                const uint32_t nt1 = (uint32_t)(shl64(tab[s][0], j) >> 32);
                const uint32_t t0 = (uint32_t)(shl64(tab[s][1], j) >> 32);
                nDm = __builtin_amdgcn_alignbit(nDm, nt1, 31);
                Xm = __builtin_amdgcn_alignbit(Xm, t0, 31);
                j -= neg_mask(nt1);
            }
            const PartEvents ev = part_events<WD_HALF>(lp, true, half == 0, ncols, nDm, Xm, nIm, j - j0, last_dx, alive);
            if constexpr (EDITS) part_edits<WD_HALF, false, 2>(a, ll, ev, lp, flush_pieces);
            else if constexpr (!NONE) part_runs<WD_HALF, 3>(ll, ev, lp, flush_pieces);
            else (void)ev;
        }
        lp.read_idx += j;
        if constexpr (EDITS) {
            window_end_bytes<false>(ll, lp);
            flush_pieces();
        }
        st_rounds++;
    }
    if (SCRG_TIMING(a) && lane == 0) atomicAdd((unsigned long long*)&a.stats[0], (unsigned long long)st_rounds);
}

hipError_t launch_align_lane_wide(const AlignArgs& a, int grid, size_t lds_bytes, hipStream_t s, LaneOutput out)
{
    const dim3 g((grid + 3) / 4), b(256);
    if (a.W <= 64) with_lane_output(out, [&](auto o) { hipLaunchKernelGGL((genasm_lane_wide_kernel<1, decltype(o)::value>), g, b, 4 * lds_bytes, s, a); });
    else with_lane_output(out, [&](auto o) { hipLaunchKernelGGL((genasm_lane_wide_kernel<2, decltype(o)::value>), g, b, 4 * lds_bytes, s, a); });
    return hipGetLastError();
}

}
```

### scrooge_amd/csrc/lane_common.h

```cpp
#pragma once

#include <hip/hip_runtime.h>
#include <stdint.h>

#include "genasm_kernels.h"
#include "genasm_device.h"
#include "text_revcomp.h"

namespace scrg {

constexpr int TT_XH  = bitop3_table([](int sum, int pv, int eq) { return (sum ^ pv) | eq; });
constexpr int TT_PH  = bitop3_table([](int mv, int xh, int pv) { return mv | ~(xh | pv); });
constexpr int TT_PVN = bitop3_table([](int mhs, int xv, int phs) { return mhs | ~(xv | phs); });
constexpr int TT_NOR3 = bitop3_table([](int a, int b, int c) { return ~(a | b | c); });
constexpr int TT_NIV  = bitop3_table([](int nv1, int v0, int stop) { return nv1 | ~v0 | stop; });
constexpr int TT_ANDN = bitop3_table([](int a, int b, int) { return a & ~b; });
constexpr int TT_BFI = bitop3_table([](int a, int b, int c) { return (a & c) | (b & ~c); });
constexpr int TT_ANDOR = bitop3_table([](int a, int b, int c) { return (a & b) | c; });
constexpr int TT_V0  = bitop3_table([](int pvn, int ph, int xh) { return pvn | ~(ph | xh); });

typedef uint32_t u32x2_t __attribute__((ext_vector_type(2)));
typedef __attribute__((address_space(3))) u32x2_t lds_u32x2_t;
__device__ __forceinline__ uint2 lds_read64(uint32_t addr)
{
    const u32x2_t v = *reinterpret_cast<const lds_u32x2_t*>((uintptr_t)addr);
    return make_uint2(v.x, v.y);
}
__device__ __forceinline__ void lds_write64(uint32_t addr, uint2 v)
{
    u32x2_t w;
    w.x = v.x;
    w.y = v.y;
    *reinterpret_cast<lds_u32x2_t*>((uintptr_t)addr) = w;
}
__device__ __forceinline__ void lds_store_u8(uint32_t addr, uint32_t v)
{
    *reinterpret_cast<volatile __attribute__((address_space(3))) uint8_t*>((uintptr_t)addr) = (uint8_t)v;
}

__device__ __forceinline__ uint32_t ffbh_u32(uint32_t v)
{
    uint32_t r;
    asm("v_ffbh_u32 %0, %1" : "=v"(r) : "v"(v));
    return r;
}

__device__ __forceinline__ uint32_t ffbl_u32(uint32_t v)
{
    uint32_t r;
    asm("v_ffbl_b32 %0, %1" : "=v"(r) : "v"(v));
    return r;
}

__device__ __forceinline__ uint32_t add_twice(uint32_t q, uint32_t bit)
{
    uint32_t r;
    asm("v_lshl_add_u32 %0, %1, 1, %2" : "=v"(r) : "v"(bit), "v"(q));
    return r;
}

__device__ __forceinline__ uint32_t mad24(uint32_t a, uint32_t b, uint32_t c)
{
    uint32_t r;
    asm("v_mad_u32_u24 %0, %1, %2, %3" : "=v"(r) : "v"(a), "s"(b), "v"(c));
    return r;
}

__device__ __forceinline__ uint32_t add3(uint32_t a, uint32_t b, uint32_t c)
{
    uint32_t r;
    asm("v_add3_u32 %0, %1, %2, %3" : "=v"(r) : "v"(a), "v"(b), "s"(c));
    return r;
}

__device__ __forceinline__ uint64_t shl64(uint64_t v, uint32_t s)
{
    uint64_t r;
    asm("v_lshlrev_b64 %0, %1, %2" : "=v"(r) : "v"(s), "v"(v));
    return r;
}
__device__ __forceinline__ uint64_t shr64(uint64_t v, uint32_t s)
{
    uint64_t r;
    asm("v_lshrrev_b64 %0, %1, %2" : "=v"(r) : "v"(s), "v"(v));
    return r;
}
__device__ __forceinline__ uint32_t clz64(uint64_t v)
{
    return min(ffbh_u32((uint32_t)(v >> 32)), ffbh_u32((uint32_t)v) + 32u);
}

__device__ __forceinline__ uint32_t hw_wave_slot()
{
    return __builtin_amdgcn_s_getreg((3 << 11) | (0 << 6) | 4);
}

__device__ __forceinline__ void rotate_priority(uint32_t round)
{
    const uint32_t pr = round & 3u;
    if (pr == 0) __builtin_amdgcn_s_setprio(0);
    else if (pr == 1) __builtin_amdgcn_s_setprio(1);
    else if (pr == 2) __builtin_amdgcn_s_setprio(2);
    else __builtin_amdgcn_s_setprio(3);
}

__device__ __forceinline__ uint32_t claim_pairs(const AlignArgs& a, uint32_t lane, bool want)
{
    const uint64_t askers = __ballot(want);
    const int first = __ffsll((unsigned long long)askers) - 1;
    uint32_t base = 0;
    if ((int)lane == first) base = atomicAdd(a.counter, (uint32_t)__popcll(askers));
    base = (uint32_t)__shfl((int)base, first);
    return base + (uint32_t)__popcll(askers & ((1ull << lane) - 1ull));
}

__device__ __forceinline__ Planes text_revcomp_word(const uint64_t* __restrict__ seq, uint64_t off, uint32_t text_len, uint32_t ref_idx,
                                                    uint32_t w, uint32_t stride)
{
    const TextRevAt r = text_rev_at(text_len, ref_idx, w);
    const Planes f = load_window_strided(seq, off, r.at, stride);
    Planes t;
    t.lo = ~brev64(f.lo << r.sh);
    t.hi = ~brev64(f.hi << r.sh);
    return t;
}

struct LanePair {
    uint64_t text_off, read_off, cigar_off;
    uint32_t text_len, read_len, cigar_cap;
    bool rev, trev;
};
__device__ __forceinline__ LanePair unpack_pair(const AlignArgs& a, uint32_t idx)
{
    const scrg_pair_desc pd = a.pairs[idx];
    LanePair p;
    const TextStretch ts = text_stretch(pd.text_off, pd.text_len, a.text_rev != 0u, a.text_stride);
    p.text_off = ts.off;
    p.trev = ts.rev;
    p.read_off = a.stranded ? pd.read_off & ~SCRG_READ_REVCOMP : pd.read_off;
    p.rev = a.stranded && (pd.read_off & SCRG_READ_REVCOMP) != 0;
    p.text_len = ts.len;
    p.read_len = (uint32_t)pd.read_len;
    p.cigar_off = pd.cigar_off;
    p.cigar_cap = pd.cigar_cap > 0xffffffffull ? 0xffffffffu : (uint32_t)pd.cigar_cap;
    return p;
}

__device__ __forceinline__ uint32_t pair_edit_limit(const AlignArgs& a, uint32_t read_len)
{
    const uint32_t by_len = a.per_mille ? (uint32_t)((uint64_t)a.per_mille * read_len / 1000u) : 0xffffffffu;
    return min(a.max_edits, by_len);
}

template <bool EDITS>
__device__ __forceinline__ void write_piece(const AlignArgs& a, const uint32_t* lds, uint32_t ring_b, uint64_t cigar_off, uint32_t cigar_cap,
                                            uint32_t& flushed, bool store = true)
{
    const uint32_t rd = EDITS ? (ring_b >> 2) + ((flushed & 32u) >> 2) : (ring_b >> 2) + ((flushed & 16u) >> 1);
    uint32_t w[8];
#pragma unroll
    for (int k = 0; k < 8; k++) w[k] = lds[rd + k];
    const bool room = EDITS ? flushed + 32u <= 2u * (uint64_t)cigar_cap : flushed + 16u <= cigar_cap;
    if (store && room) {
        uint4* const dst = EDITS ? reinterpret_cast<uint4*>(reinterpret_cast<uint8_t*>(a.runs + cigar_off) + flushed)
                                 : reinterpret_cast<uint4*>(a.runs + cigar_off + flushed);
        dst[0] = make_uint4(w[0], w[1], w[2], w[3]);
        dst[1] = make_uint4(w[4], w[5], w[6], w[7]);
    }
    flushed += EDITS ? 32u : 16u;
}

template <bool EDITS, bool PIECES = true>
__device__ __forceinline__ void retire_pair(const AlignArgs& a, const uint32_t* lds, uint32_t ring_b, uint32_t pair, uint64_t cigar_off,
                                            uint32_t cigar_cap, uint32_t& flushed, uint32_t n, int32_t nr, uint32_t edits, bool store = true)
{
    if (EDITS) {
        if (PIECES)
            while (n - flushed >= 32u) write_piece<true>(a, lds, ring_b, cigar_off, cigar_cap, flushed, store);
        const uint32_t rem = n - flushed;
        const uint32_t rd = (ring_b >> 2) + ((flushed & 32u) >> 2);
        uint32_t* const dst = reinterpret_cast<uint32_t*>(reinterpret_cast<uint8_t*>(a.runs + cigar_off) + flushed);
        for (uint32_t k = 0; 4u * k < rem; k++) {
            const uint32_t left = rem - 4u * k;
            const uint32_t keep = left >= 4u ? 0xffffffffu : (0xffffffffu >> (32u - 8u * left));
            if (flushed + 4u * k < 2u * (uint64_t)cigar_cap) dst[k] = lds[rd + k] & keep;
        }
        a.ed[pair] = (int64_t)edits;
        a.n_runs[pair] = n;
        a.status[pair] = n > 2u * (uint64_t)cigar_cap ? LANE_STATUS_OVERFLOW : LANE_STATUS_DONE;
        if (a.run_count) a.run_count[pair] = (uint32_t)(nr + 1);
    } else {
        if (PIECES)
            while (n - flushed >= 16u) write_piece<false>(a, lds, ring_b, cigar_off, cigar_cap, flushed, store);
        const uint32_t rem = n - flushed;
        const uint32_t rd = (ring_b >> 2) + ((flushed & 16u) >> 1);
        uint32_t* const dst = reinterpret_cast<uint32_t*>(a.runs + cigar_off + flushed);
        for (uint32_t k = 0; 2u * k < rem; k++)
            if (flushed + 2u * k < cigar_cap) dst[k] = lds[rd + k];
        a.ed[pair] = (int64_t)edits;
        a.n_runs[pair] = n;
        a.status[pair] = n > cigar_cap ? LANE_STATUS_OVERFLOW : LANE_STATUS_DONE;
    }
}

template <int OUT>
__device__ __forceinline__ void abandon_pair(const AlignArgs& a, uint32_t pair, uint32_t edits)
{
    a.ed[pair] = (int64_t)edits;
    if (OUT != LANE_OUT_NONE) a.n_runs[pair] = 0u;
    a.status[pair] = LANE_STATUS_OVER_EDIT_LIMIT;
    if (OUT == LANE_OUT_EDITS && a.run_count) a.run_count[pair] = 0u;
    if (OUT == LANE_OUT_NONE && a.text_end) a.text_end[pair] = 0u;
}

__device__ __forceinline__ void retire_pair_distance(const AlignArgs& a, uint32_t pair, uint32_t edits, uint32_t ref_idx)
{
    a.ed[pair] = (int64_t)edits;
    a.status[pair] = 0u;
    if (a.text_end) a.text_end[pair] = ref_idx;
}

}
```

### scrooge_amd/csrc/lane_multiword.h

```cpp
#pragma once

#include "lane_common.h"

namespace scrg {

struct LaneWork {
    bool has_pair = false;
    uint32_t pair = 0;
    uint64_t text_off = 0, read_off = 0, cigar_off = 0;
    uint32_t text_len = 0, read_len = 0, cigar_cap = 0;
    uint32_t ref_idx = 0, read_idx = 0, edits = 0;
    uint32_t lim = 0xffffffffu;
    int32_t nr = -1;
    uint32_t flushed = 0;
    uint32_t pos = 0;
    uint32_t mbase = 0;
    bool queue_empty = false;
};

template <int OUT, bool PIECES = true>
__device__ __forceinline__ bool next_pairs(const AlignArgs& a, const uint32_t* lds, uint32_t ring_b, uint32_t lane, LaneWork& w, bool& rev, bool& trev)
{
    for (;;) {
        const bool over = w.has_pair && w.edits > w.lim;
        const bool fin = over || (w.has_pair && w.read_idx >= w.read_len);
        if (__any(fin)) {
            constexpr bool EDITS = OUT == LANE_OUT_EDITS;
            if (over) abandon_pair<OUT>(a, w.pair, w.edits);
            else if constexpr (OUT == LANE_OUT_NONE) { if (fin) retire_pair_distance(a, w.pair, w.edits, w.ref_idx); }
            else if (fin) retire_pair<EDITS, PIECES>(a, lds, ring_b, w.pair, w.cigar_off, w.cigar_cap, w.flushed, EDITS ? w.pos : (uint32_t)(w.nr + 1), w.nr, w.edits);
            w.has_pair = w.has_pair && !fin;
        }
        const bool want = !w.has_pair && !w.queue_empty;
        if (!__any(want)) break;
        const uint32_t idx = claim_pairs(a, lane, want);
        const bool got = want && idx < a.n_pairs;
        if (__any(want && idx >= a.n_pairs)) w.queue_empty = true;
        if (got) {
            const LanePair p = unpack_pair(a, idx);
            w.pair = idx;
            w.text_off = p.text_off;
            w.read_off = p.read_off;
            rev = p.rev;
            trev = p.trev;
            w.text_len = p.text_len;
            w.read_len = p.read_len;
            w.lim = pair_edit_limit(a, p.read_len);
            if constexpr (OUT == LANE_OUT_NONE) {
                w.ref_idx = w.read_idx = w.edits = 0;
            } else {
                w.cigar_off = p.cigar_off;
                w.cigar_cap = p.cigar_cap;
                w.ref_idx = w.read_idx = w.edits = w.flushed = w.pos = w.mbase = 0;
                w.nr = -1;
            }
            w.has_pair = true;
        }
    }
    return __any(w.has_pair);
}

template <int NW> struct LaneVec {
    uint2 pv[NW], mv[NW];
};

template <int NW>
__device__ __forceinline__ void load_planes(const uint64_t* __restrict__ seq, uint64_t off, uint32_t k, uint32_t count, uint32_t stride,
                                            uint32_t (&lo)[2 * NW], uint32_t (&hi)[2 * NW])
{
    uint32_t s;
    const uint64_t w0 = window_first_word(off, k, stride, s);
    uint64_t v[2 * NW + 1];
#pragma unroll
    for (int q = 0; q <= 2 * NW; q++) v[q] = 32u * (uint32_t)q < s + count ? seq[w0 + (uint64_t)q * stride] : 0ull;
#pragma unroll
    for (int q = 0; q < 2 * NW; q++) {
        lo[q] = __builtin_amdgcn_alignbit((uint32_t)v[q + 1], (uint32_t)v[q], s);
        hi[q] = __builtin_amdgcn_alignbit((uint32_t)(v[q + 1] >> 32), (uint32_t)(v[q] >> 32), s);
    }
}

struct LaneWindow {
    uint32_t n;
    uint32_t m;
    uint32_t jlim;
};
__device__ __forceinline__ LaneWindow window_extent(const LaneWork& w, uint32_t W, uint32_t tbl)
{
    LaneWindow x;
    x.n = (w.has_pair && w.ref_idx < w.text_len) ? min(W, w.text_len - w.ref_idx) : 0u;
    x.m = w.has_pair ? min(W, w.read_len - w.read_idx) : 1u;
    x.jlim = w.has_pair ? min(x.m, tbl) : 0u;
    return x;
}

template <int NW, uint32_t SLOT>
__device__ __forceinline__ void window_setup(const AlignArgs& a, const LaneWork& w, bool rev, bool trev, const LaneWindow& win, uint32_t eq_b,
                                             uint32_t nomatch_b, uint32_t swz, LaneVec<NW>& st, uint32_t (&tl)[2 * NW], uint32_t (&th)[2 * NW])
{
    uint32_t plo[2 * NW], phi[2 * NW];
#pragma unroll
    for (int q = 0; q < 2 * NW; q++) { plo[q] = phi[q] = tl[q] = th[q] = 0; }
    if (w.has_pair) {
        if (!trev) load_planes<NW>(a.seq, w.text_off, w.ref_idx, win.n, a.text_stride, tl, th);
        load_planes<NW>(a.seq, w.read_off, w.read_idx, win.m, a.read_stride, plo, phi);
    }
    if (a.text_rev && __any(w.has_pair && trev)) {
#pragma unroll
        for (int q = 0; q < NW; q++) {
            if (w.has_pair && trev && 64u * (uint32_t)q < win.n) {
                const Planes tv = text_revcomp_word(a.seq, w.text_off, w.text_len, w.ref_idx, (uint32_t)q, a.text_stride);
                tl[2 * q] = (uint32_t)tv.lo; tl[2 * q + 1] = (uint32_t)(tv.lo >> 32);
                th[2 * q] = (uint32_t)tv.hi; th[2 * q + 1] = (uint32_t)(tv.hi >> 32);
            }
        }
    }
    const uint32_t x = eq_b | (swz * SLOT);
    const uint32_t m = win.m;
#pragma unroll
    for (int q = 0; q < NW; q++) {
        uint32_t rl1 = __builtin_bitreverse32(plo[2 * q]), rl0 = __builtin_bitreverse32(plo[2 * q + 1]);
        uint32_t rh1 = __builtin_bitreverse32(phi[2 * q]), rh0 = __builtin_bitreverse32(phi[2 * q + 1]);
        if (a.stranded && __any(w.has_pair && rev)) {
            const Planes rv = revcomp_pattern_word(a.seq, w.read_off, w.read_len, w.has_pair ? w.read_idx : w.read_len, (uint32_t)q, a.read_stride);
            if (w.has_pair && rev) {
                rl1 = (uint32_t)(rv.lo >> 32); rl0 = (uint32_t)rv.lo;
                rh1 = (uint32_t)(rv.hi >> 32); rh0 = (uint32_t)rv.hi;
            }
        }
        const uint32_t lo_chars = 64u * (uint32_t)q;
        const uint64_t valid = m >= lo_chars + 64u ? ~0ull : (m <= lo_chars ? 0ull : ~0ull << (64u - (m - lo_chars)));
        const uint32_t iv0 = ~(uint32_t)valid, iv1 = ~(uint32_t)(valid >> 32);
        lds_write64((x ^ (0u * SLOT)) + 8u * q, make_uint2(~(rl0 | rh0) | iv0, ~(rl1 | rh1) | iv1));
        lds_write64((x ^ (1u * SLOT)) + 8u * q, make_uint2((rl0 & ~rh0) | iv0, (rl1 & ~rh1) | iv1));
        lds_write64((x ^ (2u * SLOT)) + 8u * q, make_uint2((~rl0 & rh0) | iv0, (~rl1 & rh1) | iv1));
        lds_write64((x ^ (3u * SLOT)) + 8u * q, make_uint2((rl0 & rh0) | iv0, (rl1 & rh1) | iv1));
        lds_write64(nomatch_b + 8u * q, make_uint2(iv0, iv1));
        st.pv[q] = make_uint2((uint32_t)valid, (uint32_t)(valid >> 32));
        st.mv[q] = make_uint2(0u, 0u);
    }
    const uint32_t swl = 0u - (swz & 1u), swh = 0u - (swz >> 1);
#pragma unroll
    for (int q = 0; q < 2 * NW; q++) { tl[q] ^= swl; th[q] ^= swh; }
}

template <int NW> __device__ __forceinline__ void add_chain(const uint32_t (&a)[2 * NW], const uint32_t (&b)[2 * NW], uint32_t (&s)[2 * NW])
{
    if constexpr (NW == 1) {
        const uint64_t sum = add64(((uint64_t)a[1] << 32) | a[0], ((uint64_t)b[1] << 32) | b[0]);
        s[0] = (uint32_t)sum;
        s[1] = (uint32_t)(sum >> 32);
    } else if constexpr (NW == 2) {
        asm("v_add_co_u32 %0, vcc, %4, %8\n\t"
            "v_addc_co_u32 %1, vcc, %5, %9, vcc\n\t"
            "v_addc_co_u32 %2, vcc, %6, %10, vcc\n\t"
            "v_addc_co_u32 %3, vcc, %7, %11, vcc"
            : "=&v"(s[0]), "=&v"(s[1]), "=&v"(s[2]), "=&v"(s[3])
            : "v"(a[0]), "v"(a[1]), "v"(a[2]), "v"(a[3]), "v"(b[0]), "v"(b[1]), "v"(b[2]), "v"(b[3])
            : "vcc");
    } else if constexpr (NW == 3) {
        asm("v_add_co_u32 %0, vcc, %6, %12\n\t"
            "v_addc_co_u32 %1, vcc, %7, %13, vcc\n\t"
            "v_addc_co_u32 %2, vcc, %8, %14, vcc\n\t"
            "v_addc_co_u32 %3, vcc, %9, %15, vcc\n\t"
            "v_addc_co_u32 %4, vcc, %10, %16, vcc\n\t"
            "v_addc_co_u32 %5, vcc, %11, %17, vcc"
            : "=&v"(s[0]), "=&v"(s[1]), "=&v"(s[2]), "=&v"(s[3]), "=&v"(s[4]), "=&v"(s[5])
            : "v"(a[0]), "v"(a[1]), "v"(a[2]), "v"(a[3]), "v"(a[4]), "v"(a[5]), "v"(b[0]), "v"(b[1]), "v"(b[2]), "v"(b[3]), "v"(b[4]), "v"(b[5])
            : "vcc");
    } else {
        asm("v_add_co_u32 %0, vcc, %8, %16\n\t"
            "v_addc_co_u32 %1, vcc, %9, %17, vcc\n\t"
            "v_addc_co_u32 %2, vcc, %10, %18, vcc\n\t"
            "v_addc_co_u32 %3, vcc, %11, %19, vcc\n\t"
            "v_addc_co_u32 %4, vcc, %12, %20, vcc\n\t"
            "v_addc_co_u32 %5, vcc, %13, %21, vcc\n\t"
            "v_addc_co_u32 %6, vcc, %14, %22, vcc\n\t"
            "v_addc_co_u32 %7, vcc, %15, %23, vcc"
            : "=&v"(s[0]), "=&v"(s[1]), "=&v"(s[2]), "=&v"(s[3]), "=&v"(s[4]), "=&v"(s[5]), "=&v"(s[6]), "=&v"(s[7])
            : "v"(a[0]), "v"(a[1]), "v"(a[2]), "v"(a[3]), "v"(a[4]), "v"(a[5]), "v"(a[6]), "v"(a[7]),
              "v"(b[0]), "v"(b[1]), "v"(b[2]), "v"(b[3]), "v"(b[4]), "v"(b[5]), "v"(b[6]), "v"(b[7])
            : "vcc");
    }
}

template <int NW> struct LaneColumn {
    uint2 xh[NW], ph[NW];
};

template <int NW> __device__ __forceinline__ LaneColumn<NW> sweep_column(LaneVec<NW>& st, const uint2 (&eq)[NW])
{
    LaneColumn<NW> col;
    uint2 xv[NW], mh[NW];
    {
        uint32_t aa[2 * NW], bb[2 * NW], ss[2 * NW];
#pragma unroll
        for (int q = 0; q < NW; q++) {
            aa[2 * q] = eq[NW - 1 - q].x & st.pv[NW - 1 - q].x;
            aa[2 * q + 1] = eq[NW - 1 - q].y & st.pv[NW - 1 - q].y;
            bb[2 * q] = st.pv[NW - 1 - q].x;
            bb[2 * q + 1] = st.pv[NW - 1 - q].y;
        }
        add_chain<NW>(aa, bb, ss);
#pragma unroll
        for (int q = 0; q < NW; q++) {
            col.xh[NW - 1 - q].x = bitop3<TT_XH>(ss[2 * q], st.pv[NW - 1 - q].x, eq[NW - 1 - q].x);
            col.xh[NW - 1 - q].y = bitop3<TT_XH>(ss[2 * q + 1], st.pv[NW - 1 - q].y, eq[NW - 1 - q].y);
        }
    }
#pragma unroll
    for (int q = 0; q < NW; q++) {
        xv[q].x = eq[q].x | st.mv[q].x;
        xv[q].y = eq[q].y | st.mv[q].y;
        col.ph[q].x = bitop3<TT_PH>(st.mv[q].x, col.xh[q].x, st.pv[q].x);
        col.ph[q].y = bitop3<TT_PH>(st.mv[q].y, col.xh[q].y, st.pv[q].y);
        mh[q].x = st.pv[q].x & col.xh[q].x;
        mh[q].y = st.pv[q].y & col.xh[q].y;
    }
    uint2 phs[NW], mhs[NW];
    {
        const uint64_t p = shl1(((uint64_t)col.ph[NW - 1].y << 32) | col.ph[NW - 1].x), m = shl1(((uint64_t)mh[NW - 1].y << 32) | mh[NW - 1].x);
        phs[NW - 1] = make_uint2((uint32_t)p, (uint32_t)(p >> 32));
        mhs[NW - 1] = make_uint2((uint32_t)m, (uint32_t)(m >> 32));
    }
#pragma unroll
    for (int q = NW - 2; q >= 0; q--) {
        phs[q].x = __builtin_amdgcn_alignbit(col.ph[q].x, col.ph[q + 1].y, 31);
        phs[q].y = __builtin_amdgcn_alignbit(col.ph[q].y, col.ph[q].x, 31);
        mhs[q].x = __builtin_amdgcn_alignbit(mh[q].x, mh[q + 1].y, 31);
        mhs[q].y = __builtin_amdgcn_alignbit(mh[q].y, mh[q].x, 31);
    }
#pragma unroll
    for (int q = 0; q < NW; q++) {
        st.pv[q].x = bitop3<TT_PVN>(mhs[q].x, xv[q].x, phs[q].x);
        st.pv[q].y = bitop3<TT_PVN>(mhs[q].y, xv[q].y, phs[q].y);
        st.mv[q].x = phs[q].x & xv[q].x;
        st.mv[q].y = phs[q].y & xv[q].y;
    }
    return col;
}

template <int NW>
__device__ __forceinline__ void table_words(const LaneVec<NW>& st, const LaneColumn<NW>& col, int r, uint2 stop, uint64_t& nv1, uint64_t& v0)
{
    nv1 = ((uint64_t)bitop3<TT_NOR3>(st.pv[r].y, col.ph[r].y, stop.y) << 32) | bitop3<TT_NOR3>(st.pv[r].x, col.ph[r].x, stop.x);
    v0 = ((uint64_t)(bitop3<TT_V0>(st.pv[r].y, col.ph[r].y, col.xh[r].y) | stop.y) << 32) | (bitop3<TT_V0>(st.pv[r].x, col.ph[r].x, col.xh[r].x) | stop.x);
}

struct LaneLds {
    uint32_t* lds;
    uint32_t ring_b, scr_b;
    __device__ __forceinline__ char* bytes() const { return reinterpret_cast<char*>(lds); }
    __device__ __forceinline__ uint8_t* u8() const { return reinterpret_cast<uint8_t*>(lds); }
};

struct PartEvents {
    uint32_t ti;
    uint32_t D, X, Im;
    uint32_t B;
    uint32_t cont;
};

template <int COLS>
__device__ __forceinline__ PartEvents part_events(LaneWork& w, bool live, bool first, uint32_t ncols, uint32_t nDm, uint32_t Xm, uint32_t nIm,
                                                  uint32_t steps, uint32_t& last_dx, bool& alive)
{
    PartEvents e;
    const uint32_t nsh = 32u - ncols;
    const uint32_t Draw = ~(nDm << nsh), Xraw = Xm << nsh;
    e.ti = live ? min(ffbh_u32(Draw & Xraw), ncols) : 0u;
    const uint32_t A = ~(uint32_t)shr64(0xffffffffull, e.ti);
    e.D = Draw & A;
    e.X = Xraw & A;
    e.Im = ~nIm << nsh;
    e.B = ((e.D ^ (e.D >> 1)) | (e.X ^ (e.X >> 1)) | e.Im | 0x80000000u) & A;
    w.edits += steps - e.ti + 2u * (uint32_t)__builtin_popcount(e.D) + (uint32_t)__builtin_popcount(e.X);
    w.ref_idx += e.ti;
    e.cont = 0;
    if (!first) {
        const uint32_t first_dx = ((e.D >> 31) << 1) | (e.X >> 31);
        e.cont = (e.ti != 0u && (e.Im >> 31) == 0u && first_dx == last_dx) ? 0x80000000u : 0u;
        e.B &= ~e.cont;
    }
    constexpr uint32_t LAST = 32u - (uint32_t)COLS;
    last_dx = e.ti == (uint32_t)COLS ? ((((e.D >> LAST) & 1u) << 1) | ((e.X >> LAST) & 1u)) : 4u;
    alive = w.has_pair && e.ti == (uint32_t)COLS;
    return e;
}

template <int COLS, uint32_t TRIPS, class Flush>
__device__ __forceinline__ void part_runs(const LaneLds& l, const PartEvents& e, LaneWork& w, Flush&& flush)
{
    char* const lds_b = l.bytes();
    const uint8_t* const lds8 = l.u8();
    uint32_t E = e.B | e.Im;
    uint32_t c = ffbh_u32(E);
    if (e.cont) {
        uint16_t* const prev = reinterpret_cast<uint16_t*>(lds_b + l.ring_b + ((2u * (uint32_t)w.nr) & 62u));
        *prev = (uint16_t)(*prev + min(c, e.ti));
    }
    uint32_t ni = lds8[l.scr_b + (c & (uint32_t)(COLS - 1))];
    uint32_t nr2 = 2u * (uint32_t)w.nr;
    auto event = [&]() {
        const uint32_t sh = 31u - c;
        const uint32_t bit = 0x80000000u >> (c & 31u);
        const uint32_t live = ~c >> 31;
        *reinterpret_cast<uint16_t*>(lds_b + l.ring_b + ((nr2 + 2u) & 62u)) = (uint16_t)(((uint32_t)'I' << 8) | ni);
        nr2 += 2u * __builtin_amdgcn_ubfe(e.Im, sh, live);
        E = bitop3<TT_ANDN>(E, bit, bit);
        const uint32_t nx = ffbh_u32(E);
        ni = lds8[l.scr_b + (nx & (uint32_t)(COLS - 1))];
        const uint32_t len = min(nx, e.ti) - c;
        const uint32_t rw = (((uint32_t)'=' << 8) + len) + __builtin_amdgcn_ubfe(e.D, sh, live) * (7u << 8) + __builtin_amdgcn_ubfe(e.X, sh, live) * (27u << 8);
        *reinterpret_cast<uint16_t*>(lds_b + l.ring_b + ((nr2 + 2u) & 62u)) = (uint16_t)rw;
        nr2 += 2u * __builtin_amdgcn_ubfe(e.B, sh, live);
        c = nx;
    };
    uint32_t trips = 0;
    while (__any(E != 0u)) {
        event();
        event();
        if (++trips == TRIPS) {
            trips = 0;
            w.nr = (int32_t)nr2 >> 1;
            flush();
        }
    }
    w.nr = (int32_t)nr2 >> 1;
    flush();
}

template <int COLS, bool LONG, uint32_t TRIPS, class Flush>
__device__ __forceinline__ void part_edits(const AlignArgs& a, const LaneLds& l, const PartEvents& e, LaneWork& w, Flush&& flush)
{
    uint8_t* const lds8 = l.u8();
    uint32_t E = e.D | e.X | e.Im;
    w.nr += (int32_t)(__builtin_popcount(e.B) + __builtin_popcount(e.Im));
    uint32_t c = ffbh_u32(E);
    uint32_t ni = lds8[l.scr_b + (c & (uint32_t)(COLS - 1))];
    const uint32_t DX = e.D | e.X;
    auto put = [&](uint32_t at, uint32_t b) { lds8[l.ring_b + (at & 63u)] = (uint8_t)b; };
    auto event = [&]() {
        const uint32_t sh = 31u - c;
        const uint32_t bit = 0x80000000u >> (c & 31u);
        const uint32_t lv = ~c >> 31;
        uint32_t iB = __builtin_amdgcn_ubfe(e.Im, sh, lv), dx = __builtin_amdgcn_ubfe(DX, sh, lv);
        const uint32_t xB = __builtin_amdgcn_ubfe(e.X, sh, lv);
        const uint32_t t = w.mbase + c;
        E = bitop3<TT_ANDN>(E, bit, bit);
        const uint32_t nx = ffbh_u32(E);
        const uint32_t step = 0xC0u - 0x80u * xB;
        uint32_t k63 = 0;
        if constexpr (LONG) k63 = ((t >= 63u ? 1u : 0u) + (t >= 126u ? 1u : 0u)) * (iB | dx);
        const uint32_t r = (t - 63u * k63) & 63u;
        const bool side = max(ni * iB, 2u * k63) > 3u;
        if (__any(side)) {
            if (side) {
                auto emit = [&](uint32_t b) {
                    put(w.pos, b);
                    w.pos++;
                    if (w.pos - w.flushed >= 32u) write_piece<true>(a, l.lds, l.ring_b, w.cigar_off, w.cigar_cap, w.flushed);
                };
                for (uint32_t q = k63; q; q--) emit(0x3Fu);
                if (!LONG || iB) {
                    emit(0x80u | r);
                    for (uint32_t q = 1; q < ni; q++) emit(0x80u);
                    w.mbase = 0u - c;
                }
                if (dx) {
                    emit(step | ((!LONG || iB) ? 0u : r));
                    w.mbase = ~c;
                }
                iB = dx = k63 = 0;
            }
        }
        if constexpr (LONG) {
            put(w.pos, 0x3Fu);
            w.pos += k63;
        }
        put(w.pos, 0x80u | r);
        put(w.pos + 1u, 0x80u);
        put(w.pos + 2u, 0x80u);
        w.pos += iB ? ni : 0u;
        put(w.pos, step | (iB ? 0u : r));
        w.pos += dx;
        w.mbase = dx ? ~c : (iB ? 0u - c : w.mbase);
        ni = lds8[l.scr_b + (nx & (uint32_t)(COLS - 1))];
        c = nx;
    };
    uint32_t trips = 0;
    while (__any(E != 0u)) {
        event();
        event();
        if (++trips == TRIPS) {
            trips = 0;
            flush();
        }
    }
    flush();
    w.mbase += e.ti;
}

template <bool LONG> __device__ __forceinline__ void window_end_bytes(const LaneLds& l, LaneWork& w)
{
    uint8_t* const lds8 = l.u8();
    uint32_t k63 = w.mbase >= 63u ? 1u : 0u;
    lds8[l.ring_b + (w.pos & 63u)] = (uint8_t)0x3Fu;
    if constexpr (LONG) {
        k63 += w.mbase >= 126u ? 1u : 0u;
        lds8[l.ring_b + ((w.pos + 1u) & 63u)] = (uint8_t)0x3Fu;
    }
    w.pos += w.has_pair ? k63 : 0u;
    lds8[l.ring_b + (w.pos & 63u)] = (uint8_t)(w.mbase - 63u * k63);
    w.pos += w.has_pair ? 1u : 0u;
    w.mbase = 0;
}

}
```

Measured before the change: 78.61 million.

## Use ballot-based wave_any, pair-fuse band distance adds, drop has_pair predicates

Replaces __any with a ballot-based wave_any helper across all lane kernels. In the band table loop it pairs consecutive distance-count updates into a single v_add3_u32 and seeds the count with an initial value. In the main kernel it drops has_pair masking from many wave votes by resetting per-lane state (revm, text-rev flag, pos/nr) when a pair retires and by giving idle lanes full-size windows, and it exits the refill loop with a ballot of holders. This is meant to cut vote and predicate overhead in hot loops, but idle lanes now take part in the window and traceback work, and any state that is not reset could alter results.

```diff
diff --git a/scrooge_amd/csrc/genasm_lane_kernel.hip b/scrooge_amd/csrc/genasm_lane_kernel.hip
--- a/scrooge_amd/csrc/genasm_lane_kernel.hip
+++ b/scrooge_amd/csrc/genasm_lane_kernel.hip
@@ -137,14 +137,20 @@
 }
 constexpr bool LANE_BAND_TABLE = true;
 constexpr uint32_t BAND_STRETCH = 32, BAND_REDO_MAX = 6;
-__device__ __forceinline__ uint32_t add_masked(uint32_t acc, const uint32_t x, const uint32_t mask)
+__device__ __forceinline__ uint32_t and_masked(const uint32_t x, const uint32_t mask)
 {
     uint32_t t;
-    asm volatile("v_and_b32 %0, %2, %3\n\tv_add_u32 %1, %1, %0" : "=&v"(t), "+v"(acc) : "s"(mask), "v"(x));
+    asm volatile("v_and_b32 %0, %1, %2" : "=v"(t) : "s"(mask), "v"(x));
+    return t;
+}
+__device__ __forceinline__ uint32_t add_masked2(uint32_t acc, const uint32_t t, const uint32_t x, const uint32_t mask)
+{
+    uint32_t u;
+    asm volatile("v_and_b32 %0, %2, %3\n\tv_add3_u32 %1, %1, %4, %0" : "=&v"(u), "+v"(acc) : "s"(mask), "v"(x), "v"(t));
     return acc;
 }
-__device__ __forceinline__ uint32_t lane_window_table_band(const Planes tw, const uint64_t rlo, const uint64_t rhi, const uint32_t TBL,
-                                                           uint64_t (&tab)[LANE_TB_COLS], const uint32_t eq_b)
+__device__ __forceinline__ int32_t lane_window_table_band(const Planes tw, const uint64_t rlo, const uint64_t rhi, const uint32_t TBL,
+                                                          uint64_t (&tab)[LANE_TB_COLS], const uint32_t eq_b, const uint32_t fd0)
 {
     lane_write_eq<false>(rlo, rhi, 0u, 0u, eq_b, 0u);
     const LaneEqAddr ea(tw, eq_b);
@@ -160,7 +166,7 @@
 #pragma unroll
     for (int k = 0; k < LANE_EQ_AHEAD; k++) eqw[k] = lds_read64(ea.at(63 - k));
     uint32_t pv = ~0u << (BAND_DOWN + 1), mv = 0u;
-    uint32_t fd = 0u;
+    uint32_t fd = fd0, ft = 0u;
 #pragma unroll
     for (int i = 63; i >= 0; i--) {
         const uint32_t eq = band_eq(eqw[(63 - i) % LANE_EQ_AHEAD], i);
@@ -169,7 +175,8 @@
         const uint32_t d0 = bitop3<TT_D0>((eq & pv) + pv, pv, xv);
         const uint32_t ph = bitop3<TT_PH>(mv, d0, pv);
         const uint32_t mh = pv & d0;
-        fd = add_masked(fd, d0, 1u << (32 - BAND_UP));
+        if (i & 1) ft = and_masked(d0, 1u << (32 - BAND_UP));
+        else fd = add_masked2(fd, ft, d0, 1u << (32 - BAND_UP));
         const uint32_t xvs = xv >> 1;
         pv = bitop3<TT_PVN>(mh, xvs, ph);
         mv = ph & xvs;
@@ -181,7 +188,7 @@
             tab[i] = ((uint64_t)v1 << 32) | v0;
         }
     }
-    return 64u - (fd >> (32 - BAND_UP));
+    return 64 - (int32_t)(fd >> (32 - BAND_UP));
 }
 
 template <int OUT>
@@ -234,15 +241,15 @@
     };
     auto flush_pieces = [&]() {
         if constexpr (!NONE) {
-            const bool need = has_pair && (EDITS ? pos - flushed >= 32u : nr - (int32_t)flushed >= 15);
-            if (__any(need)) {
+            const bool need = EDITS ? pos - flushed >= 32u : nr - (int32_t)flushed >= 15;
+            if (wave_any(need)) {
                 if (need) write_piece();
             }
         }
     };
     auto ring_guard = [&](uint32_t fill, uint32_t limit) {
-        if (__any(has_pair && fill >= limit)) {
-            if (has_pair && fill >= (EDITS ? 32u : 16u)) write_piece();
+        if (wave_any(fill >= limit)) {
+            if (fill >= (EDITS ? 32u : 16u)) write_piece();
         }
     };
 
@@ -250,20 +257,31 @@
     for (;;) {
         if (!SCRG_SW(a, 1)) rotate_priority(rot++);
         const uint64_t tm0 = timing ? __builtin_readcyclecounter() : 0;
+        uint64_t holders;
         for (;;) {
             const bool over = has_pair && edits > lim;
             const bool fin = over || (has_pair && read_idx >= read_len);
-            if (__any(fin)) {
-                if (over) abandon_pair<OUT>(a, pair, edits);
-                else if constexpr (NONE) { if (fin) retire_pair_distance(a, pair, edits, ref_idx); }
+            if (wave_any(fin)) {
+                if (over) {
+                    abandon_pair<OUT>(a, pair, edits);
+                    if constexpr (!NONE) {
+                        flushed = pos = 0;
+                        nr = -1;
+                    }
+                } else if constexpr (NONE) { if (fin) retire_pair_distance(a, pair, edits, ref_idx); }
                 else if (fin) retire_pair<EDITS>(a, lds, ring_b, pair, cigar_off, cigar_cap, flushed, EDITS ? pos : (uint32_t)(nr + 1), nr, edits, !SCRG_ABL(a, 16));
                 has_pair = has_pair && !fin;
-            }
-            const bool want = !has_pair && !queue_empty;
-            if (!__any(want)) break;
+                if (fin) {
+                    revm = 0u;
+                    tr_in &= ~LANE_TEXT_REV;
+                }
+            }
+            holders = __builtin_amdgcn_ballot_w64(has_pair);
+            if (queue_empty || holders == ~0ull) break;
+            const bool want = !has_pair;
             const uint32_t idx = claim_pairs(a, lane, want);
             const bool got = want && idx < a.n_pairs;
-            if (__any(want && idx >= a.n_pairs)) queue_empty = true;
+            if (wave_any(want && idx >= a.n_pairs)) queue_empty = true;
             if (got) {
                 const scrg_pair_desc pd = a.pairs[idx];
                 pair = idx;
@@ -289,13 +307,13 @@
                 pwords = load_window_words_at(read_w, tr_in >> 8, lane_read_offset(0u, 0u, read_len, revm), a.read_stride);
             }
         }
-        if (!__any(has_pair)) break;
-        const bool wave_rev = a.stranded && __any(has_pair && revm != 0u);
-        const bool wave_trev = a.text_rev && __any(has_pair && (tr_in & LANE_TEXT_REV) != 0u);
+        if (holders == 0ull) break;
+        const bool wave_rev = a.stranded && wave_any(revm != 0u);
+        const bool wave_trev = a.text_rev && wave_any((tr_in & LANE_TEXT_REV) != 0u);
 
         const uint64_t tm1 = timing ? __builtin_readcyclecounter() : 0;
-        const uint32_t n = has_pair ? min(W, sub_sat_u32(text_len, ref_idx)) : 0u;
-        const uint32_t m = has_pair ? min(W, read_len - read_idx) : 1u;
+        const uint32_t n = has_pair ? min(W, sub_sat_u32(text_len, ref_idx)) : 64u;
+        const uint32_t m = has_pair ? min(W, read_len - read_idx) : 64u;
         Planes tw = window_planes(twords);
         const Planes pw = window_planes(pwords);
         if (wave_trev) lane_text_rev(tw, text_len, ref_idx, tr_in);
@@ -306,7 +324,7 @@
         uint64_t tab[LANE_TB_COLS];
         const uint32_t jlim = has_pair ? min(m, TBL) : 0u;
         const uint32_t stop = 0x80000000u >> jlim;
-        const bool short_n = __any(has_pair && n != 64u);
+        const bool short_n = wave_any(n != 64u);
         uint64_t rlo, rhi;
         lane_pattern_rev(pw, read_len - read_idx, revm, wave_rev, rlo, rhi);
         uint32_t j = 0, ti, nDm = 0, Xm = 0, nIm = 0;
@@ -334,13 +352,13 @@
         bool walked = false, eq_written = false;
         uint64_t tm3 = 0;
         if constexpr (BAND) {
-            if (W == 64u && !short_n && !__any(has_pair && m != 64u) && !SCRG_SEL(a.debug, SCRG_SWITCH_NO_BAND) && !SCRG_ABL(a, 2) && !SCRG_ABL(a, 8)) {
+            if (W == 64u && !short_n && !wave_any(m != 64u) && !SCRG_SEL(a.debug, SCRG_SWITCH_NO_BAND) && !SCRG_ABL(a, 2) && !SCRG_ABL(a, 8)) {
                 if ((band_ctl >> 16) != 0u) {
                     band_ctl -= 1u << 16;
                     st_skipped++;
                 } else {
-                    const uint32_t d_band = lane_window_table_band(tw, rlo, rhi, TBL, tab, eq_b);
-                    walked = !__any(has_pair && d_band > (uint32_t)BAND_SAFE);
+                    const int32_t d_band = lane_window_table_band(tw, rlo, rhi, TBL, tab, eq_b, stop & 0x80000000u);
+                    walked = !wave_any(d_band > BAND_SAFE);
                     eq_written = true;
                     st_band++;
                     st_redone += walked ? 0u : 1u;
@@ -417,7 +435,7 @@
                     const uint32_t nx = ffbh_u32(E);
                     const uint32_t step = 0xC0u - 0x80u * xB;
                     const bool side = ni * iB > 3u;
-                    if (__any(side)) {
+                    if (wave_any(side)) {
                         if (side) {
                             auto emit = [&](uint32_t b) {
                                 put(pos, b);
@@ -445,7 +463,7 @@
                     c = nx;
                 };
                 uint32_t trips = 0;
-                while (__any(E != 0u)) {
+                while (wave_any(E != 0u)) {
                     if (trips >= 2u) ring_guard(pos - flushed, 50u);
                     event();
                     event();
@@ -478,8 +496,8 @@
                 event(c0, n0, c1);
                 event(c1, n1, c0);
             };
-            for (uint32_t trips = 0; trips < 4u && __any(c0 < 32u); trips++) trip();
-            while (__any(c0 < 32u)) {
+            for (uint32_t trips = 0; trips < 4u && wave_any(c0 < 32u); trips++) trip();
+            while (wave_any(c0 < 32u)) {
                 ring_guard((q >> 1) - flushed, 27u);
                 trip();
             }
@@ -566,10 +584,10 @@
                 has_pair = has_pair && read_idx < read_len && edits <= lim;
                 for (;;) {
                     const bool want = !has_pair && !queue_empty;
-                    if (!__any(want)) break;
+                    if (!wave_any(want)) break;
                     const uint32_t idx = claim_pairs(a, lane, want);
                     const bool got = want && idx < a.n_pairs;
-                    if (__any(want && idx >= a.n_pairs)) queue_empty = true;
+                    if (wave_any(want && idx >= a.n_pairs)) queue_empty = true;
                     if (got) {
                         const LanePair p = unpack_pair(a, idx);
                         pair = idx;
@@ -587,7 +605,7 @@
                         pwords = load_window_words(a.seq, read_off, lane_read_offset(0u, 0u, read_len, revm), a.read_stride);
                     }
                 }
-                if (!__any(has_pair)) active = false;
+                if (!wave_any(has_pair)) active = false;
             }
             if (active) {
                 const bool live = has_pair && read_idx < read_len;
@@ -598,13 +616,13 @@
                     tw = window_planes(twords);
                     pw = window_planes(pwords);
                 }
-                const bool wave_trev = a.text_rev && __any(live && trev);
+                const bool wave_trev = a.text_rev && wave_any(live && trev);
                 if (wave_trev) lane_text_rev(tw, text_len, ref_idx, trev ? LANE_TEXT_REV : 0u);
                 uint64_t tab[LANE_TB_COLS];
                 const uint32_t jlim = live ? min(m, TBL) : 0u;
                 const uint32_t stop = 0x80000000u >> jlim;
-                const bool short_n = __any(live && n != 64u);
-                const bool wave_rev = a.stranded && __any(live && revm != 0u);
+                const bool short_n = wave_any(live && n != 64u);
+                const bool wave_rev = a.stranded && wave_any(live && revm != 0u);
                 uint64_t rlo, rhi;
                 lane_pattern_rev(pw, read_len - read_idx, revm, wave_rev, rlo, rhi);
                 if (short_n) lane_window_table<true>(tw, rlo, rhi, n, m, stop, tab, eq_b, nomatch_b);
@@ -670,13 +688,13 @@
     uint32_t flushed = 0;
     auto flush_pieces = [&]() {
         const bool need = open && nr - (int32_t)flushed >= 16;
-        if (__any(need)) {
+        if (wave_any(need)) {
             if (need) write_piece<false>(a, lds, ring_b, cigar_off, cigar_cap, flushed);
         }
     };
     auto consume = [&](uint32_t buf) {
         const uint32_t meta = lds[rec_w(buf, 3)];
-        if (!__any((meta & SPLIT_VALID) != 0u)) return;
+        if (!wave_any((meta & SPLIT_VALID) != 0u)) return;
         const bool valid = (meta & SPLIT_VALID) != 0u;
         const uint32_t ti = meta & 31u;
         const uint32_t D = valid ? lds[rec_w(buf, 0)] : 0u, X = valid ? lds[rec_w(buf, 1)] : 0u, Im = valid ? lds[rec_w(buf, 2)] : 0u;
@@ -711,7 +729,7 @@
             c = nx;
         };
         uint32_t trips = 0;
-        while (__any(E != 0u)) {
+        while (wave_any(E != 0u)) {
             event();
             event();
             if (++trips == 3u) {
@@ -723,7 +741,7 @@
         nr = ((int32_t)q >> 1) - 1;
         flush_pieces();
         const bool fin = valid && (meta & SPLIT_LAST) != 0u;
-        if (__any(fin)) {
+        if (wave_any(fin)) {
             if (fin && (meta & SPLIT_OVER)) {
                 abandon_pair<LANE_OUT_RUNS>(a, pair, lds[rec_w(buf, 5)]);
                 open = false;
diff --git a/scrooge_amd/csrc/genasm_lane_mw_kernel.hip b/scrooge_amd/csrc/genasm_lane_mw_kernel.hip
--- a/scrooge_amd/csrc/genasm_lane_mw_kernel.hip
+++ b/scrooge_amd/csrc/genasm_lane_mw_kernel.hip
@@ -38,7 +38,7 @@
     auto flush_pieces = [&]() {
         for (;;) {
             const bool need = lp.has_pair && lp.nr + 1 - (int32_t)lp.flushed >= 16;
-            if (!__any(need)) break;
+            if (!wave_any(need)) break;
             if (need) write_piece();
         }
     };
@@ -58,7 +58,7 @@
         const uint32_t n = (lp.has_pair && lp.ref_idx < lp.text_len) ? min(W, lp.text_len - lp.ref_idx) : 0u;
         const uint32_t m = lp.has_pair ? min(W, lp.read_len - lp.read_idx) : 1u;
         uint64_t tlo[NW], thi[NW], rlo[NW], rhi[NW], valid[NW];
-        const bool wave_trev = a.text_rev && __any(lp.has_pair && trev);
+        const bool wave_trev = a.text_rev && wave_any(lp.has_pair && trev);
 #pragma unroll
         for (int w = 0; w < NW; w++) {
             Planes t = {0, 0}, p = {0, 0};
@@ -71,7 +71,7 @@
             thi[w] = t.hi;
             rlo[w] = brev64(p.lo);
             rhi[w] = brev64(p.hi);
-            if (a.stranded && __any(lp.has_pair && rev)) {
+            if (a.stranded && wave_any(lp.has_pair && rev)) {
                 const Planes rv = revcomp_pattern_word(a.seq, lp.read_off, lp.read_len, lp.has_pair ? lp.read_idx : lp.read_len, (uint32_t)w, a.read_stride);
                 if (lp.has_pair && rev) { rlo[w] = rv.lo; rhi[w] = rv.hi; }
             }
@@ -189,7 +189,7 @@
 #pragma unroll
                 for (int r = 0; r < RW; r++) Ev.w[r] = D.w[r] | X.w[r] | Im.w[r];
                 lp.nr += (int32_t)(row_pop<RW>(B) + row_pop<RW>(Im));
-                while (__any(row_any<RW>(Ev))) {
+                while (wave_any(row_any<RW>(Ev))) {
                     if (row_any<RW>(Ev)) {
                         const uint32_t c = row_clz<RW>(Ev);
                         const Row<RW> bit = row_bit<RW>(c);
@@ -212,7 +212,7 @@
                         }
                     }
                 }
-                if (__any(lp.has_pair)) {
+                if (wave_any(lp.has_pair)) {
                     if (lp.has_pair) {
                         uint32_t t = lp.mbase + ti;
                         for (; t >= 63u; t -= 63u) emit(0x3Fu);
@@ -221,7 +221,7 @@
                 }
                 lp.mbase = 0;
             } else
-            while (__any(row_any<RW>(E))) {
+            while (wave_any(row_any<RW>(E))) {
                 if (row_any<RW>(E)) {
                     const uint32_t c = row_clz<RW>(E);
                     if (row_test<RW>(Im, c)) push_run((uint32_t)'I', lds8[len_b + c]);
diff --git a/scrooge_amd/csrc/genasm_lane_parts_kernel.hip b/scrooge_amd/csrc/genasm_lane_parts_kernel.hip
--- a/scrooge_amd/csrc/genasm_lane_parts_kernel.hip
+++ b/scrooge_amd/csrc/genasm_lane_parts_kernel.hip
@@ -100,7 +100,7 @@
     auto flush_pieces = [&]() {
         if constexpr (!NONE) for (;;) {
             const bool need = lp.has_pair && (EDITS ? lp.pos - lp.flushed >= 32u : lp.nr - (int32_t)lp.flushed >= 16);
-            if (!__any(need)) break;
+            if (!wave_any(need)) break;
             if (need) write_piece<EDITS>(a, lds, ring_b, lp.cigar_off, lp.cigar_cap, lp.flushed);
         }
     };
@@ -154,7 +154,7 @@
         auto sweep_chunk = [&](int32_t k, auto store_tag) {
             constexpr bool STORE = decltype(store_tag)::value;
             const int32_t nrel = (int32_t)n - (int32_t)PT_COLS * k;
-            if (!__any(has_pair && nrel > 0)) {
+            if (!wave_any(has_pair && nrel > 0)) {
                 if (STORE) {
                     LaneVec<NW> keep = st;
                     pt_sweep16<NW, true, true>(keep, 0u, 0u, nrel, stop, tab, eq_b, nomatch_b);
@@ -164,7 +164,7 @@
             const uint2 xx = lds_read64(text_b + 8u * (uint32_t)(k >> 1));
             const uint32_t sh = (uint32_t)(k & 1) * 16u;
             const uint32_t xe = xx.x >> sh, xo = xx.y >> sh;
-            if (__any(has_pair && nrel < PT_COLS)) pt_sweep16<NW, STORE, true>(st, xe, xo, nrel, stop, tab, eq_b, nomatch_b);
+            if (wave_any(has_pair && nrel < PT_COLS)) pt_sweep16<NW, STORE, true>(st, xe, xo, nrel, stop, tab, eq_b, nomatch_b);
             else pt_sweep16<NW, STORE, false>(st, xe, xo, nrel, stop, tab, eq_b, nomatch_b);
         };
 #pragma unroll 1
@@ -183,7 +183,7 @@
         for (uint32_t part = 0; part < P; part++) {
             const uint32_t ncols = min((uint32_t)PT_COLS, TBL - (uint32_t)PT_COLS * part);
             if (part != 0u) {
-                if (!__any(alive)) break;
+                if (!wave_any(alive)) break;
                 if (!PREFETCH) load_checkpoint(part, st);
                 sweep_chunk((int32_t)part, std::true_type{});
                 if (PREFETCH && part + 1u < P) load_checkpoint(part + 1u, st);
@@ -236,11 +236,11 @@
             };
             if (TBL <= 63u) {
                 walk_part(std::integral_constant<int, 1>{});
-            } else if (!__any(has_pair && j0 < 64u)) {
+            } else if (!wave_any(has_pair && j0 < 64u)) {
                 walk_part(std::integral_constant<int, 2>{});
-            } else if (!__any(has_pair && j0 > 40u)) {
+            } else if (!wave_any(has_pair && j0 > 40u)) {
                 walk_part(std::integral_constant<int, 1>{});
-                if (__any(has_pair && j > 63u)) walk_part(std::integral_constant<int, 0>{});
+                if (wave_any(has_pair && j > 63u)) walk_part(std::integral_constant<int, 0>{});
             } else {
                 walk_part(std::integral_constant<int, 0>{});
             }
diff --git a/scrooge_amd/csrc/genasm_lane_wide_kernel.hip b/scrooge_amd/csrc/genasm_lane_wide_kernel.hip
--- a/scrooge_amd/csrc/genasm_lane_wide_kernel.hip
+++ b/scrooge_amd/csrc/genasm_lane_wide_kernel.hip
@@ -110,7 +110,7 @@
     auto flush_pieces = [&]() {
         if constexpr (!NONE) for (;;) {
             const bool need = lp.has_pair && (EDITS ? lp.pos - lp.flushed >= 32u : lp.nr - (int32_t)lp.flushed >= 16);
-            if (!__any(need)) break;
+            if (!wave_any(need)) break;
             if (need) write_piece<EDITS>(a, lds, ring_b, lp.cigar_off, lp.cigar_cap, lp.flushed);
         }
     };
@@ -129,8 +129,8 @@
         win.stop = make_uint2((uint32_t)stop64, (uint32_t)(stop64 >> 32));
         LaneVec<NW> st0;
         window_setup<NW, 8u * NW>(a, lp, rev, trev, ext, eq_b, nomatch_b, swz, st0, win.tl, win.th);
-        const bool short_n = __any(has_pair && n < 64u);
-        const bool short_pro = NW == 2 && __any(has_pair && n != ((W + 15u) & ~15u));
+        const bool short_n = wave_any(has_pair && n < 64u);
+        const bool short_pro = NW == 2 && wave_any(has_pair && n != ((W + 15u) & ~15u));
         uint64_t tab[WD_HALF][2];
         if constexpr (NW == 2) {
             if (W <= 80u) {
@@ -154,7 +154,7 @@
 #pragma unroll 1
         for (int half = 0; half < 2; half++) {
             const uint32_t ncols = half == 0 ? (uint32_t)WD_HALF : HB;
-            if (half == 1 && (HB == 0u || !__any(alive))) break;
+            if (half == 1 && (HB == 0u || !wave_any(alive))) break;
             {
                 LaneVec<NW> st = st0;
                 if (half == 0) {
diff --git a/scrooge_amd/csrc/lane_common.h b/scrooge_amd/csrc/lane_common.h
--- a/scrooge_amd/csrc/lane_common.h
+++ b/scrooge_amd/csrc/lane_common.h
@@ -88,6 +88,11 @@
 __device__ __forceinline__ uint32_t clz64(uint64_t v)
 {
     return min(ffbh_u32((uint32_t)(v >> 32)), ffbh_u32((uint32_t)v) + 32u);
+}
+
+__device__ __forceinline__ bool wave_any(bool pred)
+{
+    return __builtin_amdgcn_ballot_w64(pred) != 0ull;
 }
 
 __device__ __forceinline__ uint32_t hw_wave_slot()
diff --git a/scrooge_amd/csrc/lane_multiword.h b/scrooge_amd/csrc/lane_multiword.h
--- a/scrooge_amd/csrc/lane_multiword.h
+++ b/scrooge_amd/csrc/lane_multiword.h
@@ -24,7 +24,7 @@
     for (;;) {
         const bool over = w.has_pair && w.edits > w.lim;
         const bool fin = over || (w.has_pair && w.read_idx >= w.read_len);
-        if (__any(fin)) {
+        if (wave_any(fin)) {
             constexpr bool EDITS = OUT == LANE_OUT_EDITS;
             if (over) abandon_pair<OUT>(a, w.pair, w.edits);
             else if constexpr (OUT == LANE_OUT_NONE) { if (fin) retire_pair_distance(a, w.pair, w.edits, w.ref_idx); }
@@ -32,10 +32,10 @@
             w.has_pair = w.has_pair && !fin;
         }
         const bool want = !w.has_pair && !w.queue_empty;
-        if (!__any(want)) break;
+        if (!wave_any(want)) break;
         const uint32_t idx = claim_pairs(a, lane, want);
         const bool got = want && idx < a.n_pairs;
-        if (__any(want && idx >= a.n_pairs)) w.queue_empty = true;
+        if (wave_any(want && idx >= a.n_pairs)) w.queue_empty = true;
         if (got) {
             const LanePair p = unpack_pair(a, idx);
             w.pair = idx;
@@ -57,7 +57,7 @@
             w.has_pair = true;
         }
     }
-    return __any(w.has_pair);
+    return wave_any(w.has_pair);
 }
 
 template <int NW> struct LaneVec {
@@ -105,7 +105,7 @@
         if (!trev) load_planes<NW>(a.seq, w.text_off, w.ref_idx, win.n, a.text_stride, tl, th);
         load_planes<NW>(a.seq, w.read_off, w.read_idx, win.m, a.read_stride, plo, phi);
     }
-    if (a.text_rev && __any(w.has_pair && trev)) {
+    if (a.text_rev && wave_any(w.has_pair && trev)) {
 #pragma unroll
         for (int q = 0; q < NW; q++) {
             if (w.has_pair && trev && 64u * (uint32_t)q < win.n) {
@@ -121,7 +121,7 @@
     for (int q = 0; q < NW; q++) {
         uint32_t rl1 = __builtin_bitreverse32(plo[2 * q]), rl0 = __builtin_bitreverse32(plo[2 * q + 1]);
         uint32_t rh1 = __builtin_bitreverse32(phi[2 * q]), rh0 = __builtin_bitreverse32(phi[2 * q + 1]);
-        if (a.stranded && __any(w.has_pair && rev)) {
+        if (a.stranded && wave_any(w.has_pair && rev)) {
             const Planes rv = revcomp_pattern_word(a.seq, w.read_off, w.read_len, w.has_pair ? w.read_idx : w.read_len, (uint32_t)q, a.read_stride);
             if (w.has_pair && rev) {
                 rl1 = (uint32_t)(rv.lo >> 32); rl0 = (uint32_t)rv.lo;
@@ -317,7 +317,7 @@
         c = nx;
     };
     uint32_t trips = 0;
-    while (__any(E != 0u)) {
+    while (wave_any(E != 0u)) {
         event();
         event();
         if (++trips == TRIPS) {
@@ -354,7 +354,7 @@
         if constexpr (LONG) k63 = ((t >= 63u ? 1u : 0u) + (t >= 126u ? 1u : 0u)) * (iB | dx);
         const uint32_t r = (t - 63u * k63) & 63u;
         const bool side = max(ni * iB, 2u * k63) > 3u;
-        if (__any(side)) {
+        if (wave_any(side)) {
             if (side) {
                 auto emit = [&](uint32_t b) {
                     put(w.pos, b);
@@ -389,7 +389,7 @@
         c = nx;
     };
     uint32_t trips = 0;
-    while (__any(E != 0u)) {
+    while (wave_any(E != 0u)) {
         event();
         event();
         if (++trips == TRIPS) {
```

Result: faster. 79.46 million (median of 6 runs) (+1.1%).
